# zacharie12/Hypernet-image-captioning

Hardware: AMD Instinct MI355X
Metric: training images/sec at 1/2/4/8 MI355X, Flickr30k GRU+hypernet bs=128 (higher is better)
Workload: dtype f32; 1 GPU; Flickr30k-shaped GRU+additive-attention decoder + hypernet (3 style domains), full training step (fwd, CE, bwd, clip 5.0, Adam); per_gpu_batch=128, global_batch=128, T=20, P=49, D=2048, F=200, E=200, H=200, V=9684, hypernet_params=144906720, parallelism=dp1, launch=eager, next_theta_in_adam_pass=True, next_precompute_beside_adam=True, spinup_steps=0, deterministic_gradients=True

## Files before the change

### hypernet-image-captioning_amd/caphn/_lib.py

```python
import ctypes as C
import os

import torch

_HERE = os.path.dirname(os.path.abspath(__file__))
LIB_PATH = os.environ.get("CAPHN_LIB_PATH") or os.path.join(_HERE, "libcaphn.so")
MAX_HEADS = 8

c_fp = C.c_void_p


class HyperDesc(C.Structure):
    _fields_ = [("he", C.c_int), ("n_heads", C.c_int),
                ("k", C.c_int * MAX_HEADS), ("w", C.c_int * MAX_HEADS),
                ("base_w0", c_fp), ("base_b0", c_fp), ("base_w2", c_fp), ("base_b2", c_fp),
                ("w1", c_fp * MAX_HEADS), ("b1", c_fp * MAX_HEADS),
                ("w2", c_fp * MAX_HEADS), ("b2", c_fp * MAX_HEADS),
                ("d_in", C.c_int), ("d_mid", C.c_int)]


class HyperGrads(C.Structure):
    _fields_ = [("g_base_w0", c_fp), ("g_base_b0", c_fp), ("g_base_w2", c_fp), ("g_base_b2", c_fp),
                ("g_w1", c_fp * MAX_HEADS), ("g_b1", c_fp * MAX_HEADS),
                ("g_w2", c_fp * MAX_HEADS), ("g_b2", c_fp * MAX_HEADS),
# ... 82 lines not shown
    "caphn_colsum_workspace_bytes": (C.c_size_t, [C.c_int, C.c_int]),
    "caphn_linear_wgrad_f32": (C.c_int, [C.c_int, C.c_int, C.c_int, c_fp, C.c_int, c_fp, C.c_int, c_fp, C.c_int, c_fp, c_fp, c_fp]),
    "caphn_colsum_f32": (C.c_int, [C.c_int, C.c_int, c_fp, C.c_int, c_fp, c_fp, c_fp]),
    "caphn_hyper_acts_floats": (C.c_int, [C.POINTER(HyperDesc)]),
    "caphn_hyper_forward": (C.c_int, [C.POINTER(HyperDesc), c_fp, c_fp, c_fp, c_fp]),
    "caphn_hyper_backward_workspace_bytes": (C.c_size_t, [C.POINTER(HyperDesc)]),
    "caphn_hyper_backward": (C.c_int, [C.POINTER(HyperDesc), c_fp, c_fp, C.POINTER(HyperGrads), c_fp, c_fp]),
    "caphn_decoder_workspace_bytes": (C.c_size_t, [C.POINTER(DecoderDims)]),
    "caphn_decoder_forward": (C.c_int, [C.POINTER(DecoderDims), C.POINTER(DecoderParams), c_fp, c_fp,
                                        c_fp, c_fp, c_fp, c_fp]),
    "caphn_decoder_pair_prep": (C.c_int, [C.POINTER(DecoderDims), C.POINTER(DecoderParams), c_fp, c_fp]),
    "caphn_decoder_pair_pack_desc": (C.c_int, [C.POINTER(DecoderDims), c_fp, C.POINTER(PairPack)]),
    "caphn_decoder_precompute": (C.c_int, [C.POINTER(DecoderDims), C.POINTER(DecoderParams), c_fp, c_fp, c_fp, c_fp]),
    "caphn_decoder_inputs": (C.c_int, [C.POINTER(DecoderDims), C.POINTER(DecoderParams), c_fp, c_fp, c_fp]),
    "caphn_decoder_lookup": (C.c_int, [C.POINTER(DecoderDims), C.POINTER(DecoderParams), c_fp, c_fp, c_fp]),
    "caphn_decoder_prepare_rows": (C.c_int, [C.POINTER(DecoderDims), c_fp, C.c_int64, c_fp, c_fp]),
    "caphn_decoder_forward_sampled": (C.c_int, [C.POINTER(DecoderDims), C.POINTER(DecoderParams), c_fp, c_fp,
                                                C.c_char_p, c_fp, c_fp, c_fp, c_fp]),
    "caphn_decoder_forward_sampled_train": (C.c_int, [C.POINTER(DecoderDims), C.POINTER(DecoderParams), c_fp, c_fp,
                                                      C.c_char_p, c_fp, c_fp, c_fp, c_fp]),
    "caphn_decoder_backward": (C.c_int, [C.POINTER(DecoderDims), C.POINTER(DecoderParams), c_fp, c_fp,
                                         c_fp, c_fp, C.POINTER(DecoderGrads), c_fp, c_fp]),
    "caphn_decoder_hyper_backward": (C.c_int, [C.POINTER(DecoderDims), C.POINTER(DecoderParams), c_fp, c_fp,
                                               c_fp, c_fp, C.POINTER(DecoderGrads), c_fp,
                                               C.POINTER(HyperDesc), c_fp, C.POINTER(HyperGrads), c_fp, c_fp]),
    "caphn_decoder_backward_milestone": (C.c_int, [C.c_int, c_fp]),
    "caphn_decoder_search_workspace_bytes": (C.c_size_t, [C.POINTER(DecoderDims), C.POINTER(SearchCfg)]),
    "caphn_decoder_search_begin": (C.c_int, [C.POINTER(DecoderDims), C.POINTER(DecoderParams), C.POINTER(SearchCfg),
                                             c_fp, c_fp, c_fp, c_fp]),
    "caphn_decoder_search_steps": (C.c_int, [C.POINTER(DecoderDims), C.POINTER(DecoderParams), C.POINTER(SearchCfg),
                                             C.c_int, C.c_int, c_fp, c_fp, c_fp, c_fp]),
    "caphn_decoder_search_result": (C.c_int, [C.POINTER(DecoderDims), C.POINTER(SearchCfg), C.c_int, c_fp, c_fp,
                                              c_fp, c_fp, c_fp, c_fp, c_fp, c_fp]),
    "caphn_plain_workspace_bytes": (C.c_size_t, [C.POINTER(PlainDims)]),
    "caphn_plain_forward": (C.c_int, [C.POINTER(PlainDims), C.POINTER(PlainParams), c_fp, c_fp, c_fp, c_fp, c_fp, c_fp, c_fp]),
    "caphn_bahdanau_fwd": (C.c_int, [C.c_int] * 4 + [c_fp] * 8),
    "caphn_bahdanau_bwd": (C.c_int, [C.c_int] * 4 + [c_fp] * 12),
    "caphn_plain_forward_sampled": (C.c_int, [C.POINTER(PlainDims), C.POINTER(PlainParams), c_fp, c_fp, c_fp, C.c_uint64, c_fp, c_fp,
                                               c_fp, c_fp]),
    "caphn_plain_backward": (C.c_int, [C.POINTER(PlainDims), C.POINTER(PlainParams), c_fp, c_fp, c_fp, c_fp, c_fp,
                                       C.POINTER(PlainGrads), c_fp, c_fp]),
    "caphn_layernorm_fwd": (C.c_int, [C.c_int, C.c_int, c_fp, c_fp, c_fp, C.c_float, c_fp, c_fp, c_fp, c_fp]),
    "caphn_layernorm_bwd_workspace_bytes": (C.c_size_t, [C.c_int, C.c_int]),
    "caphn_layernorm_bwd": (C.c_int, [C.c_int, C.c_int, c_fp, c_fp, c_fp, c_fp, c_fp, c_fp, c_fp, c_fp, c_fp, c_fp]),
    "caphn_attention_supported": (C.c_int, [C.POINTER(AttnDims)]),
    "caphn_attention_fwd": (C.c_int, [C.POINTER(AttnDims), c_fp, c_fp, c_fp, c_fp, c_fp, c_fp, c_fp, c_fp]),
    "caphn_attention_bwd": (C.c_int, [C.POINTER(AttnDims), c_fp, c_fp, c_fp, c_fp, c_fp, c_fp, c_fp, c_fp, c_fp, c_fp, c_fp, c_fp]),
    "caphn_ce_workspace_bytes": (C.c_size_t, [C.c_int]),
    "caphn_cross_entropy_rows": (C.c_int, [C.c_int, C.c_int, c_fp, c_fp, C.c_int64, c_fp, C.c_int, c_fp, c_fp, c_fp]),
    "caphn_cross_entropy_rows_ld": (C.c_int, [C.c_int, C.c_int, C.c_int, c_fp, c_fp, C.c_int64, c_fp, C.c_int, c_fp, c_fp, c_fp]),
    "caphn_cross_entropy_finish": (C.c_int, [C.c_int, c_fp, c_fp, c_fp, c_fp]),
    "caphn_decoder_profile_ptr": (C.c_void_p, [C.POINTER(DecoderDims), c_fp]),
    "caphn_decoder_rowcount_ptr": (C.c_void_p, [C.POINTER(DecoderDims), c_fp]),
    "caphn_cross_entropy_fwd_bwd": (C.c_int, [C.c_int, C.c_int, c_fp, c_fp, C.c_int64, c_fp, c_fp, C.c_int, c_fp, c_fp]),
    "caphn_embedding_gather": (C.c_int, [C.c_int, C.c_int, c_fp, c_fp, c_fp, c_fp]),
    "caphn_embedding_scatter_add": (C.c_int, [C.c_int, C.c_int, c_fp, c_fp, c_fp, c_fp]),
    "caphn_embedding_scatter_add_v": (C.c_int, [C.c_int, C.c_int, C.c_int, c_fp, c_fp, c_fp, c_fp]),
    "caphn_sumsq_blocks": (C.c_int, [C.c_size_t]),
    "caphn_sumsq_f32": (C.c_int, [C.c_size_t, c_fp, c_fp, c_fp]),
    "caphn_rank_sumsq_f32": (C.c_int, [C.c_int, C.c_int, C.c_int, c_fp, C.c_size_t, c_fp, C.c_size_t,
                                       c_fp, c_fp, c_fp]),
    "caphn_rank_sumsq_multi_f32": (C.c_int, [C.c_int, C.c_int, C.POINTER(C.c_int), C.POINTER(C.c_int),
                                             C.POINTER(C.c_void_p), C.POINTER(C.c_size_t), C.POINTER(C.c_void_p),
                                             C.POINTER(C.c_size_t), c_fp, c_fp, c_fp]),
    "caphn_grad_norm_workspace_bytes": (C.c_size_t, [C.c_size_t, C.c_int, C.c_int]),
    "caphn_grad_norm_coef": (C.c_int, [C.c_size_t, c_fp, C.c_int, C.c_int, C.POINTER(C.c_int), C.POINTER(C.c_int),
                                       C.POINTER(C.c_void_p), C.POINTER(C.c_size_t), C.POINTER(C.c_void_p),
                                       C.POINTER(C.c_size_t), C.c_double, C.c_double, c_fp, c_fp, c_fp]),
    "caphn_clip_coef": (C.c_int, [C.c_int, c_fp, c_fp, C.c_double, C.c_double, c_fp, c_fp]),
    "caphn_adam_dense_f32": (C.c_int, [C.c_size_t, c_fp, c_fp, c_fp, c_fp, c_fp, C.POINTER(AdamHParams), c_fp]),
    "caphn_grad_norm_adam_dense": (C.c_int, [C.c_size_t, c_fp, c_fp, c_fp, c_fp, C.c_int, C.c_int, C.POINTER(C.c_int), C.POINTER(C.c_int),
                                             C.POINTER(C.c_void_p), C.POINTER(C.c_size_t), C.POINTER(C.c_void_p), C.POINTER(C.c_size_t),
                                             C.c_double, C.c_double, c_fp, c_fp, C.POINTER(AdamHParams), C.c_int, c_fp, c_fp, c_fp, c_fp]),
    "caphn_grad_norm_multi_workspace_bytes": (C.c_size_t, [C.c_int, C.POINTER(C.c_size_t), C.c_int, C.c_int]),
    "caphn_grad_norm_multi": (C.c_int, [C.c_int, C.POINTER(C.c_void_p), C.POINTER(C.c_size_t), C.c_int, C.c_int,
                                        C.POINTER(C.c_int), C.POINTER(C.c_int), C.POINTER(C.c_void_p), C.POINTER(C.c_size_t),
                                        C.POINTER(C.c_void_p), C.POINTER(C.c_size_t), C.c_double, C.c_double, c_fp, c_fp, c_fp]),
    "caphn_adam_multi_f32": (C.c_int, [C.c_int, C.POINTER(C.c_void_p), C.POINTER(C.c_void_p), C.POINTER(C.c_void_p),
                                       C.POINTER(C.c_void_p), C.POINTER(C.c_size_t), c_fp, C.POINTER(AdamHParams), c_fp]),
    "caphn_adam_rank_f32": (C.c_int, [C.c_int, C.c_int, C.c_int, c_fp, c_fp, c_fp, c_fp, C.c_size_t,
                                      c_fp, C.c_size_t, c_fp, C.POINTER(AdamHParams), c_fp]),
    "caphn_adam_rank_gemv_f32": (C.c_int, [C.c_int, C.c_int, C.c_int, c_fp, c_fp, c_fp, c_fp, C.c_size_t,
                                           c_fp, C.c_size_t, c_fp, C.POINTER(AdamHParams), c_fp, c_fp, c_fp, c_fp]),
    "caphn_adam_rank_multi_f32": (C.c_int, [C.c_int, C.c_int, C.POINTER(RankJob), c_fp, C.POINTER(AdamHParams), c_fp]),
    "caphn_hyper_forward_acts": (C.c_int, [C.POINTER(HyperDesc), c_fp, c_fp, c_fp]),
    "caphn_stream_copy_f32": (C.c_int, [C.c_size_t, c_fp, c_fp, c_fp]),
    "caphn_outer_f32": (C.c_int, [C.c_int, C.c_int, c_fp, c_fp, c_fp, c_fp]),
    "caphn_tune": (C.c_int, [C.c_int, C.c_int]),
}

_ERR = {-1: "CAPHN_EINVAL (bad argument)", -2: "CAPHN_ELAUNCH (HIP launch error)",
        -3: "CAPHN_ELIMIT (problem exceeds a hardware limit, e.g. 160 KB LDS)",
        -4: "CAPHN_ETIMEOUT (a recurrent kernel's partner workgroup never answered: that step's results are NaN; "
            "sticky until caphn_device_error(1))"}

_lib = None


class CaphnError(RuntimeError):
    pass


def load():
    global _lib
    if _lib is not None:
        return _lib
# ... 34 lines not shown
```

### hypernet-image-captioning_amd/caphn/ops.py

```python
import ctypes as C
from dataclasses import dataclass
from typing import Dict, List, Optional, Sequence, Tuple

import torch

from . import _lib as L

GEMM_BIAS, GEMM_RELU, GEMM_ACCUM, GEMM_MASK, GEMM_LRELU = 1, 2, 4, 8, 16


def _f32(*shape, device):
    return torch.empty(*shape, dtype=torch.float32, device=device)


def gemm(a: torch.Tensor, b: torch.Tensor, ta: bool = False, tb: bool = False,
         bias: Optional[torch.Tensor] = None, relu: bool = False, out: Optional[torch.Tensor] = None,
         accumulate: bool = False, mask: Optional[torch.Tensor] = None, splitk: int = 1, lrelu: bool = False) -> torch.Tensor:
    lib = L.load()
    assert a.dim() == 2 and b.dim() == 2 and a.stride(1) == 1 and b.stride(1) == 1
    M, K = (a.shape[1], a.shape[0]) if ta else (a.shape[0], a.shape[1])
    N, Kb = (b.shape[0], b.shape[1]) if tb else (b.shape[1], b.shape[0])
    if K != Kb:
        raise L.CaphnError(f"gemm inner dims differ: {K} vs {Kb}")
    if out is None:
# ... 522 lines not shown
    lib = L.load()
    cd = dims.c()
    ps = _dec_struct(L.DecoderParams, dims, params)
    gs = _dec_struct(L.DecoderGrads, dims, grads)
    L.check(lib.caphn_decoder_backward(C.byref(cd), C.byref(ps), L.ptr(features), L.ptr(captions, torch.int64),
                                       L.ptr(dlogits), L.ptr(dalphas, allow_none=True), C.byref(gs),
                                       C.c_void_p(ws.data_ptr()), L.stream_ptr()), "caphn_decoder_backward")


def cross_entropy_fwd_bwd(logits: torch.Tensor, targets: torch.Tensor, ignore_index: int = 0,
                          dlogits: Optional[torch.Tensor] = None, leave_ignored_rows: bool = False):
    lib = L.load()
    V = logits.shape[-1]
    rows = logits.numel() // V
    if dlogits is None:
        dlogits = torch.empty_like(logits)
    ws = torch.empty(lib.caphn_ce_workspace_bytes(rows), dtype=torch.uint8, device=logits.device)
    out = _f32(2, device=logits.device)
    L.check(lib.caphn_cross_entropy_fwd_bwd(rows, V, L.ptr(logits), L.ptr(targets.reshape(-1), torch.int64),
                                            ignore_index, L.ptr(dlogits), L.ptr(out), int(leave_ignored_rows),
                                            C.c_void_p(ws.data_ptr()),
                                            L.stream_ptr()), "caphn_cross_entropy_fwd_bwd")
    return out, dlogits


def cross_entropy_rows(logits: torch.Tensor, targets: torch.Tensor, ignore_index: int, dlogits: torch.Tensor,
                       ws: torch.Tensor, leave_ignored_rows: bool = False, n_valid_ptr: Optional[int] = None, V: Optional[int] = None) -> None:
    lib = L.load()
    ld = logits.shape[-1]
    rows = logits.numel() // ld
    V = ld if V is None else int(V)
    assert dlogits.shape[-1] == ld and V <= ld
    L.check(lib.caphn_cross_entropy_rows_ld(rows, V, ld, L.ptr(logits), L.ptr(targets.reshape(-1), torch.int64), ignore_index,
                                            L.ptr(dlogits), int(leave_ignored_rows),
                                            C.c_void_p(n_valid_ptr) if n_valid_ptr else None, C.c_void_p(ws.data_ptr()),
                                            L.stream_ptr()), "caphn_cross_entropy_rows_ld")


def cross_entropy_finish(rows: int, ws: torch.Tensor, out: torch.Tensor, n_valid_ptr: Optional[int] = None) -> None:
    lib = L.load()
    L.check(lib.caphn_cross_entropy_finish(rows, C.c_void_p(n_valid_ptr) if n_valid_ptr else None, L.ptr(out),
                                           C.c_void_p(ws.data_ptr()), L.stream_ptr()), "caphn_cross_entropy_finish")


def ce_workspace(rows: int, device) -> torch.Tensor:
    return torch.empty(L.load().caphn_ce_workspace_bytes(rows), dtype=torch.uint8, device=device)


def decoder_rowcount_ptr(dims: DecDims, ws: torch.Tensor) -> int:
    cd = dims.c()
    return int(L.load().caphn_decoder_rowcount_ptr(C.byref(cd), C.c_void_p(ws.data_ptr())) or 0)


def embedding_gather(table: torch.Tensor, idx: torch.Tensor) -> torch.Tensor:
    lib = L.load()
    rows, E = idx.numel(), table.shape[1]
    out = _f32(rows, E, device=table.device)
    L.check(lib.caphn_embedding_gather(rows, E, L.ptr(table), L.ptr(idx.reshape(-1), torch.int64), L.ptr(out),
                                       L.stream_ptr()), "caphn_embedding_gather")
    return out


def embedding_scatter_add(g: torch.Tensor, idx: torch.Tensor, table_grad: torch.Tensor) -> None:
    lib = L.load()
    rows, E = g.shape
    L.check(lib.caphn_embedding_scatter_add_v(rows, E, int(table_grad.shape[0]), L.ptr(g), L.ptr(idx.reshape(-1), torch.int64),
                                              L.ptr(table_grad), L.stream_ptr()), "caphn_embedding_scatter_add_v")


def sumsq_partials(x: torch.Tensor, partial: Optional[torch.Tensor] = None) -> torch.Tensor:
    lib = L.load()
    nb = lib.caphn_sumsq_blocks(x.numel())
    if partial is None:
        partial = torch.empty(nb, dtype=torch.float64, device=x.device)
    L.check(lib.caphn_sumsq_f32(x.numel(), L.ptr(x), L.ptr(partial, torch.float64), L.stream_ptr()), "caphn_sumsq_f32")
    return partial[:nb]


def rank_sumsq(gfac: torch.Tensor, afac: torch.Tensor, acc: torch.Tensor) -> None:
    lib = L.load()
    R, rows = gfac.shape
    k = afac.shape[1]
    ws = torch.empty(2 * R * R, dtype=torch.float64, device=gfac.device)
    L.check(lib.caphn_rank_sumsq_f32(R, rows, k, gfac.data_ptr(), gfac.stride(0), afac.data_ptr(), afac.stride(0),
                                     L.ptr(acc, torch.float64), L.ptr(ws, torch.float64), L.stream_ptr()),
            "caphn_rank_sumsq_f32")


def rank_sumsq_multi(pairs, acc: torch.Tensor, ws: Optional[torch.Tensor] = None) -> None:
    lib = L.load()
    n = len(pairs)
    R = pairs[0][0].shape[0]
    if ws is None:
        ws = torch.empty(2 * R * R * n, dtype=torch.float64, device=acc.device)
    rows = (C.c_int * n)(*[g.shape[1] for g, _ in pairs])
    ks = (C.c_int * n)(*[a.shape[1] for _, a in pairs])
    gp = (C.c_void_p * n)(*[g.data_ptr() for g, _ in pairs])
    ap = (C.c_void_p * n)(*[a.data_ptr() for _, a in pairs])
    ldg = (C.c_size_t * n)(*[g.stride(0) for g, _ in pairs])
    lda = (C.c_size_t * n)(*[a.stride(0) for _, a in pairs])
    L.check(lib.caphn_rank_sumsq_multi_f32(R, n, rows, ks, gp, ldg, ap, lda, L.ptr(acc, torch.float64),
                                           L.ptr(ws, torch.float64), L.stream_ptr()), "caphn_rank_sumsq_multi_f32")


class GradNorm:

# ... 409 lines not shown
```

### hypernet-image-captioning_amd/csrc/decoder.hip

```cpp
#include "common.h"
#include "decoder_internal.h"
#include "gemm_internal.h"
#include <algorithm>
#include <initializer_list>
#include <mutex>

int g_tune_deterministic = 0;
int g_tune_rec_pair = 1;
int g_tune_rec_rotate = 1;
int g_tune_vocab_order = 1;
int g_tune_branch_mask = 7;
int g_tune_splitk_target = 1280;
int g_tune_chain_main = 0;
int g_tune_hops = 0;
int g_tune_fork = 4;
int g_tune_join_chain = 0;
int g_tune_sk_dhs = 0, g_tune_sk_vocab_w = 0;
#define RUN(x) do { int _rc = (x); if (_rc != CAPHN_OK) return _rc; } while (0)

namespace {

struct Side {
    hipStream_t st[3];
    enum { D_FORK = 0, D_JOIN = 1, D_X = 4, D_MS = 10, D_PRE_F = 14, D_PRE_ALL = 15, D_COUNT = 16 };
    struct Dep { hipEvent_t ev; unsigned seq = 0; bool by_value = false; };
    Dep deps[D_COUNT];
    unsigned* vals = nullptr;
    unsigned counter = 0;
    bool values = false;
    bool pre_valid = false;
    const void* pre_ws = nullptr;
    bool ready = false, on = false;
    bool forked[3] = {false, false, false};
    hipStream_t main = nullptr;
    int init() {
        if (ready) return CAPHN_OK;
        static std::mutex mu;
        std::lock_guard<std::mutex> lock(mu);
        if (ready) return CAPHN_OK;
        for (auto& s : st) if (hipStreamCreateWithFlags(&s, hipStreamNonBlocking) != hipSuccess) return CAPHN_ELAUNCH;
        for (auto& d : deps) if (hipEventCreateWithFlags(&d.ev, hipEventDisableTiming) != hipSuccess) return CAPHN_ELAUNCH;
        void* p = nullptr;
        if (hipMalloc(&p, sizeof(unsigned) * D_COUNT) == hipSuccess && hipMemset(p, 0, sizeof(unsigned) * D_COUNT) == hipSuccess)
            vals = static_cast<unsigned*>(p);
        else (void)hipGetLastError();
        ready = true;
        return CAPHN_OK;
    }
    int post(int slot, hipStream_t from) {
        Dep& d = deps[slot];
        if (values) {
            d.seq = ++counter; d.by_value = true;
            return hipStreamWriteValue32(from, vals + slot, d.seq, 0) == hipSuccess ? CAPHN_OK : CAPHN_ELAUNCH;
        }
        d.by_value = false;
        return hipEventRecord(d.ev, from) == hipSuccess ? CAPHN_OK : CAPHN_ELAUNCH;
    }
    int await(int slot, hipStream_t to) {
        Dep& d = deps[slot];
        if (d.by_value)
            return hipStreamWaitValue32(to, vals + slot, d.seq, hipStreamWaitValueGte, 0xffffffffu) == hipSuccess ? CAPHN_OK : CAPHN_ELAUNCH;
        return hipStreamWaitEvent(to, d.ev, 0) == hipSuccess ? CAPHN_OK : CAPHN_ELAUNCH;
    }
    int milestone(int k, hipStream_t from) {
        if (init() != CAPHN_OK) return CAPHN_ELAUNCH;
        return post(D_MS + k, from);
    }
    int begin(hipStream_t m, bool enable) {
// ... 16 lines not shown
        if (post(D_FORK, main) != CAPHN_OK) return CAPHN_ELAUNCH;
        for (int i : ids) {
            if (!((g_tune_branch_mask >> i) & 1)) continue;
            if (await(D_FORK, st[i]) != CAPHN_OK) return CAPHN_ELAUNCH;
            forked[i] = true;
        }
        return CAPHN_OK;
    }
    int jointo(int i) {
        if (!on || !((g_tune_branch_mask >> i) & 1)) return CAPHN_OK;
        forked[i] = false;
        if (post(D_JOIN + i, st[i]) != CAPHN_OK) return CAPHN_ELAUNCH;
        return await(D_JOIN + i, main);
    }
    int join_into(int i, int j) {
        if (!on || !((g_tune_branch_mask >> i) & 1)) return CAPHN_OK;
        if (!((g_tune_branch_mask >> j) & 1)) return jointo(i);
        forked[i] = false;
        if (post(D_JOIN + i, st[i]) != CAPHN_OK) return CAPHN_ELAUNCH;
        return await(D_JOIN + i, st[j]);
    }
    struct Scope {
        Side& s;
        explicit Scope(Side& side) : s(side) {}
        ~Scope() { for (int i = 0; i < 3; ++i) if (s.on && s.forked[i]) (void)s.jointo(i); }
    };
    hipStream_t xfrom[6] = {nullptr, nullptr, nullptr, nullptr, nullptr, nullptr};
    int record(int k, hipStream_t from) {
        if (!on) return CAPHN_OK;
        xfrom[k] = from;
        return post(D_X + k, from);
    }
    int wait(int k, hipStream_t to) {
        if (!on || xfrom[k] == to) return CAPHN_OK;
        return await(D_X + k, to);
    }
    int dep(hipStream_t from, hipStream_t to, int k) {
        if (!on || from == to) return CAPHN_OK;
        if (post(D_X + k, from) != CAPHN_OK) return CAPHN_ELAUNCH;
        return await(D_X + k, to);
    }
};
constexpr int MAX_DEVICES = 64;
Side g_sides[MAX_DEVICES];
inline Side* side_here() {
    int dev = 0;
    if (hipGetDevice(&dev) != hipSuccess || dev < 0 || dev >= MAX_DEVICES) return nullptr;
    return &g_sides[dev];
}

struct Ws {
    size_t Y1, f, meanf, h0, c0, Waf, G, Xe, Xg, Hs, Hprev, gates, hn, Cs, Cprev, uah, alphas, idx;
    size_t dHs, dgi, dgh, duah, de, dh0, dc0, ctx, dctx, dXe, dWaf, dmeanf, df, dY1, apart, vtmp, colws, colws_s[3], prof, rowmap;
    size_t xch, xch_floats;
    size_t wp;
    size_t H0s, dH0, h0L, dcarry, tgi, tgh, tmpA, tmpB;
    size_t Lin[CAPHN_MAX_DEC_LAYERS - 1], Lgates[CAPHN_MAX_DEC_LAYERS - 1], Lhn[CAPHN_MAX_DEC_LAYERS - 1],
           Ldgi[CAPHN_MAX_DEC_LAYERS - 1], Ldgh[CAPHN_MAX_DEC_LAYERS - 1];
    int L1;
    size_t total;
    int npc, pchunk, NG, arows;
};
inline bool use_pair(const caphn_decoder_dims* d) {
    const int NG = d->cell == CAPHN_CELL_LSTM ? 4 : 3;
    return g_tune_rec_pair && d->T > 1 && d->layers <= 1 && caphn_rec_pair_resident_gates(d->P, d->H, NG) >= 0;
}

inline size_t up4(size_t v) { return (v + 3) & ~(size_t)3; }

inline Ws layout(const caphn_decoder_dims* d) {
    Ws w;
    const size_t B = d->B, T = d->T, P = d->P, F = d->F, E = d->E, H = d->H, V = d->V, D = d->D;
    const bool lstm = d->cell == CAPHN_CELL_LSTM, raw = d->raw_features != 0;
    const size_t NG = lstm ? 4 : 3;
    w.NG = (int)NG;
    size_t o = 0;
    auto take = [&](size_t n) { size_t r = o; o += up4(n); return r; };
    w.Y1 = take(raw ? 0 : B * P * F); w.f = take(raw ? 0 : B * P * F); w.meanf = take(B * F); w.h0 = take(B * H);
    w.c0 = take(lstm ? B * H : 0);
    w.Waf = take(B * P * H); w.G = take(B * P * NG * H); w.Xe = take(B * T * (E + F)); w.Xg = take(B * T * NG * H);
    w.Hs = take(B * T * H); w.Hprev = take(B * T * H); w.gates = take(B * T * NG * H); w.hn = take(lstm ? 0 : B * T * H);
    w.Cs = take(lstm ? B * T * H : 0); w.Cprev = take(lstm ? B * T * H : 0);
    w.uah = take(B * T * H); w.alphas = take(B * T * P); w.idx = take(2 * B * T);
    w.dHs = take(B * T * H); w.dgi = take(B * T * NG * H); w.dgh = take(lstm ? 0 : B * T * NG * H); w.duah = take(B * T * H);
    w.de = take(B * T * P); w.dh0 = take(B * H); w.dc0 = take(lstm ? B * H : 0);
    w.ctx = w.Xe + E; w.dctx = take(raw ? 0 : B * T * F);
    w.dXe = take(B * T * E); w.dWaf = take(B * P * H); w.dmeanf = take(raw ? 0 : 2 * B * F); w.df = take(raw ? 0 : B * P * F);
    w.dY1 = take(raw ? 0 : B * P * F);
    w.pchunk = 1; w.npc = (int)((P + w.pchunk - 1) / w.pchunk);
    const size_t arows = std::max<size_t>(std::max<size_t>(w.npc, (size_t)caphn_rec_bwd_groups((int)P, (int)H)),
                                          (size_t)caphn_rec_pair_bwd_groups((int)P, (int)H));
    w.arows = (int)arows;
    w.apart = take(B * arows * (H + 1)); w.vtmp = take(H + 1);
    size_t cs = 0;
    auto need = [&](size_t M, size_t N) { cs = std::max(cs, caphn_colsum_workspace_bytes((int)M, (int)N) / sizeof(float)); };
    need(B * T, V); need(B * T, NG * H); need(B * T, H); need(B * P, H); need(B * P, F); need(B, H);
    need(B * arows, H + 1);
    if (d->layers > 1) need(B * (T + 1), 3 * H);
    w.colws = take(cs);
    {
        size_t c2 = 0;
        auto need2 = [&](size_t M, size_t N) { c2 = std::max(c2, caphn_colsum_workspace_bytes((int)M, (int)N) / sizeof(float)); };
        need2(B * T, NG * H); need2(B * T, H); need2(B * P, H); need2(B * P, F); need2(B, H); need2(B * arows, H + 1);
        if (d->layers > 1) need2(B * (T + 1), 3 * H);
        for (int i = 0; i < 3; ++i) w.colws_s[i] = take(c2);
    }
    w.prof = take(64);
    w.rowmap = take(B * T + 4);
    w.xch_floats = caphn_rec_pair_xch_bytes((int)B, (int)P, (int)H) / sizeof(float);
    w.xch = take(2 * w.xch_floats);
    o = (o + 31) & ~(size_t)31;
    w.wp = take(caphn_rec_pair_wp_floats((int)H, (int)NG));
    w.L1 = d->layers > 1 ? d->layers - 1 : 0;
    {
        const size_t on = w.L1 > 0 ? 1 : 0, S = T + 1;
        w.H0s = take(on * B * T * H); w.dH0 = take(on * B * T * H); w.h0L = take(on * B * H); w.dcarry = take(on * B * H);
        w.tgi = take(on * B * 3 * H); w.tgh = take(on * B * 3 * H); w.tmpA = take(on * B * H); w.tmpB = take(on * B * H);
        for (int l = 0; l < CAPHN_MAX_DEC_LAYERS - 1; ++l) {
            const size_t u = l < w.L1 ? 1 : 0;
            w.Lin[l] = take(u * B * S * H); w.Lgates[l] = take(u * B * S * 3 * H); w.Lhn[l] = take(u * B * S * H);
            w.Ldgi[l] = take(u * B * S * 3 * H); w.Ldgh[l] = take(u * B * S * 3 * H);
        }
    }
    w.total = o;
    (void)D;
    return w;
}

__global__ __launch_bounds__(1024) void valid_rows_kernel(int n, const int64_t* __restrict__ tgt, int64_t ignore, int* __restrict__ map) {
    __shared__ int wsum[16];
    __shared__ int base_s;
    const int tid = threadIdx.x, lane = tid & 63, wave = tid >> 6;
    if (tid == 0) base_s = 0;
    __syncthreads();
    for (int c0 = 0; c0 < n; c0 += 1024) {
        const int i = c0 + tid;
        const int v = (i < n && tgt[i] != ignore) ? 1 : 0;
        const unsigned long long ball = __ballot(v);
        const int before = __popcll(ball & ((1ull << lane) - 1ull));
        if (lane == 0) wsum[wave] = __popcll(ball);
        __syncthreads();
        int woff = 0, tot = 0;
        for (int q = 0; q < 16; ++q) { if (q < wave) woff += wsum[q]; tot += wsum[q]; }
        const int base = base_s;
        if (v) map[4 + base + woff + before] = i;
        __syncthreads();
        if (tid == 0) base_s = base + tot;
        __syncthreads();
    }
    if (tid == 0) map[0] = base_s;
}

__global__ void copy2_kernel(const float* __restrict__ src, int n, float* __restrict__ a, float* __restrict__ b) {
    const int i = blockIdx.x * blockDim.x + threadIdx.x;
    if (i < n) a[i] = src[i];
    else if (i == n) b[0] = src[n];
}

__global__ __launch_bounds__(256) void teacher_inputs_kernel(int T, int E, const int64_t* __restrict__ caps, const float* __restrict__ table,
                                                            int64_t* __restrict__ idx, float* __restrict__ out, int ostride) {
    const int i = blockIdx.x, t = i % T;
    const int64_t id = t < 2 ? (int64_t)-1 : caps[i - 1];
    if (threadIdx.x == 0) idx[i] = id;
    for (int e = threadIdx.x; e < E; e += 256) out[(size_t)i * ostride + e] = id < 0 ? 0.f : table[(size_t)id * E + e];
}

inline bool dims_ok(const caphn_decoder_dims* d) {
    if (d && !(d->dropout_p >= 0.f && d->dropout_p < 1.f)) return false;
    if (!(d && d->B > 0 && d->T > 0 && d->P > 0 && d->D > 0 && d->F > 0 && d->E > 0 && d->H > 0 && d->V > 0)) return false;
    if (d->cell != CAPHN_CELL_GRU && d->cell != CAPHN_CELL_LSTM) return false;
    if (d->raw_features && d->F != d->D) return false;
    if (d->layers < 0 || d->layers > CAPHN_MAX_DEC_LAYERS) return false;
    if (d->layers > 1 && d->cell != CAPHN_CELL_GRU) return false;
    if (d->logits_ld != 0 && d->logits_ld < d->V) return false;
    return true;
}
inline bool layer_params_ok(const caphn_decoder_dims* d, const caphn_decoder_params* p) {
    for (int l = 0; l + 1 < d->layers; ++l)
        if (!p->lw_ih[l] || !p->lw_hh[l] || !p->lb_ih[l] || !p->lb_hh[l]) return false;
    return true;
}

inline int pick_splitk(int M, int N, int K) {
    if (g_tune_deterministic) return 1;
    const long t128 = (long)((M + 127) / 128) * ((N + 127) / 128);
    if (t128 >= 1024) return 1;
    const long t64 = (long)((M + 63) / 64) * ((N + 63) / 64);
    const int nslab = (K + 31) / 32;
    long s = (g_tune_splitk_target + t64 - 1) / t64;
    if (s > nslab / 8) s = nslab / 8;
    if (s < 1) s = 1;
    if (s > 64) s = 64;
    return (int)s;
}


inline int gemm_auto(int ta, int tb, int M, int N, int K, const float* A, int lda, const float* B, int ldb,
                     float* C, int ldc, const float* bias, int flags, hipStream_t s,
                     const int* rowmap = nullptr, int map_mode = 0, bool prezeroed = false) {
    int sk = pick_splitk(M, N, K);
    if (rowmap) {
        if (sk > 1 && !prezeroed) {
            if (ldc == N) { RUN(caphn_zero_f32(C, (size_t)M * N, s)); }
// ... 80 lines not shown
    const int B = d->B, H = d->H, G3 = 3 * d->H;
    const float* in = hin; int in_ld = hin_ld;
    for (int l = 0; l < w.L1; ++l) {
        const bool last = l == w.L1 - 1;
        float* out = last ? hout : ws + ((l & 1) ? w.tmpB : w.tmpA);
        const int out_ld = last ? hout_ld : H;
        RUN(caphn_gemm_f32(0, 1, B, G3, H, in, in_ld, p->lw_ih[l], H, ws + w.tgi, G3, p->lb_ih[l], nullptr, 0, CAPHN_GEMM_BIAS, 1, s));
        RUN(caphn_gemm_f32(0, 1, B, G3, H, in, in_ld, p->lw_hh[l], H, ws + w.tgh, G3, p->lb_hh[l], nullptr, 0, CAPHN_GEMM_BIAS, 1, s));
        LayerFwdArgs a;
        a.B = B; a.H = H; a.S = d->T + 1; a.slot = slot;
        a.gi = ws + w.tgi; a.gh = ws + w.tgh; a.hin = in; a.hin_ld = in_ld; a.hout = out; a.hout_ld = out_ld;
        a.sin = ws + w.Lin[l]; a.sgates = ws + w.Lgates[l]; a.shn = ws + w.Lhn[l];
        if (last && slot > 0) { a.drop_p = d->dropout_p; a.drop_seed = d->dropout_seed; a.T = d->T; a.t = slot - 1; }
        RUN(caphn_launch_layer_gru_fwd(a, s));
        in = out; in_ld = out_ld;
    }
    return CAPHN_OK;
}

static int layers_backward(const caphn_decoder_dims* d, const caphn_decoder_params* p, const Ws& w, float* ws, int slot,
                           const float* d1, int d1_ld, const float* d2, float* dout, int dout_ld, hipStream_t s) {
    const int B = d->B, H = d->H, G3 = 3 * d->H, S = d->T + 1;
    for (int l = w.L1 - 1; l >= 0; --l) {
        float* o = l == 0 ? dout : ws + ((l & 1) ? w.tmpB : w.tmpA);
        const int o_ld = l == 0 ? dout_ld : H;
        LayerBwdArgs a;
        a.B = B; a.H = H; a.S = S; a.slot = slot;
        a.d1 = d1; a.d1_ld = d1_ld; a.d2 = d2;
        a.sin = ws + w.Lin[l]; a.sgates = ws + w.Lgates[l]; a.shn = ws + w.Lhn[l];
        a.dgi = ws + w.Ldgi[l]; a.dgh = ws + w.Ldgh[l]; a.dout = o; a.dout_ld = o_ld;
        if (l == w.L1 - 1 && slot > 0) { a.drop_p = d->dropout_p; a.drop_seed = d->dropout_seed; a.T = d->T; a.t = slot - 1; }
        RUN(caphn_launch_layer_gru_bwd(a, s));
        RUN(caphn_gemm_f32(0, 0, B, H, G3, ws + w.Ldgi[l] + (size_t)slot * G3, S * G3, p->lw_ih[l], H, o, o_ld, nullptr, nullptr, 0,
                           CAPHN_GEMM_ACCUM, 1, s));
        RUN(caphn_gemm_f32(0, 0, B, H, G3, ws + w.Ldgh[l] + (size_t)slot * G3, S * G3, p->lw_hh[l], H, o, o_ld, nullptr, nullptr, 0,
                           CAPHN_GEMM_ACCUM, 1, s));
        d1 = o; d1_ld = o_ld; d2 = nullptr;
    }
    return CAPHN_OK;
}

}

extern "C" size_t caphn_decoder_workspace_bytes(const caphn_decoder_dims* d) {
    if (!dims_ok(d)) return 0;
    return layout(d).total * sizeof(float);
}

extern "C" const int* caphn_decoder_rowcount_ptr(const caphn_decoder_dims* d, void* ws_) {
    if (!dims_ok(d) || !ws_) return nullptr;
    return reinterpret_cast<const int*>(static_cast<float*>(ws_) + layout(d).rowmap);
}

extern "C" unsigned long long* caphn_decoder_profile_ptr(const caphn_decoder_dims* d, void* ws_) {
    if (!dims_ok(d) || !ws_) return nullptr;
    return reinterpret_cast<unsigned long long*>(static_cast<float*>(ws_) + layout(d).prof);
}

extern "C" int caphn_decoder_prepare_rows(const caphn_decoder_dims* d, const int64_t* targets, int64_t ignore_index,
                                          void* ws_, caphn_stream_t stream) {
    if (!dims_ok(d) || !targets || !ws_) return CAPHN_EINVAL;
    const Ws w = layout(d);
    hipLaunchKernelGGL(valid_rows_kernel, dim3(1), dim3(1024), 0, static_cast<hipStream_t>(stream), d->B * d->T, targets,
                       ignore_index, reinterpret_cast<int*>(static_cast<float*>(ws_) + w.rowmap));
    return caphn_launch_status();
}

static int decoder_inputs(const caphn_decoder_dims* d, const caphn_decoder_params* p, const Ws& w, float* ws,
                          const int64_t* captions, hipStream_t s, int parts = 3) {
    const int BT = d->B * d->T, E = d->E, GH = w.NG * d->H, EF = d->E + d->F;
    int64_t* idx = reinterpret_cast<int64_t*>(ws + w.idx);
    if ((parts & 1) && !(d->precomputed & 64))
        hipLaunchKernelGGL(teacher_inputs_kernel, dim3(BT), dim3(256), 0, s, d->T, E, captions, p->embed_w, idx, ws + w.Xe, EF);
    if (parts & 2)
    RUN(caphn_gemm_f32(0, 1, BT, GH, E, ws + w.Xe, EF, p->w_ih, EF, ws + w.Xg, GH, p->b_ih, nullptr, 0, CAPHN_GEMM_BIAS, 1, s));
    return CAPHN_OK;
}

extern "C" int caphn_decoder_precompute(const caphn_decoder_dims* d, const caphn_decoder_params* p, const float* features,
                                        const int64_t* captions, void* ws_, caphn_stream_t stream) {
    if (!dims_ok(d) || !p || !features || !ws_) return CAPHN_EINVAL;
    const bool raw = d->raw_features != 0;
    if (!raw && (!p->fc0_w || !p->fc0_b || !p->fc2_w || !p->fc2_b)) return CAPHN_EINVAL;
    if (d->cell == CAPHN_CELL_LSTM && (!p->initc_w || !p->initc_b)) return CAPHN_EINVAL;
    const Ws w = layout(d);
    hipStream_t s = static_cast<hipStream_t>(stream);
    const float* f = nullptr;
    RUN(decoder_precompute(d, p, w, static_cast<float*>(ws_), features, &f, s, (captions ? 3 : 1) & ~(d->precomputed & 1), true));
    if (captions && !(d->precomputed & 4)) RUN(decoder_inputs(d, p, w, static_cast<float*>(ws_), captions, s));
    Side* sd = side_here();
    if (!sd || sd->post(Side::D_PRE_ALL, s) != CAPHN_OK) return CAPHN_ELAUNCH;
    sd->pre_valid = true;
    sd->pre_ws = ws_;
    return caphn_launch_status();
}

extern "C" int caphn_decoder_pair_prep(const caphn_decoder_dims* d, const caphn_decoder_params* p, void* ws_, caphn_stream_t stream) {
    if (!dims_ok(d) || !p || !ws_ || !p->Ua_w || !use_pair(d)) return CAPHN_EINVAL;
    const Ws w = layout(d);
    float* ws = static_cast<float*>(ws_);
    RUN(caphn_launch_rec_pair_prep(reinterpret_cast<unsigned long long*>(ws + w.xch), 2 * w.xch_floats * sizeof(float) / sizeof(unsigned long long),
                                   p->Ua_w, nullptr, d->H, w.NG, ws + w.wp, ws + w.dHs, (size_t)d->B * d->T * d->H,
                                   static_cast<hipStream_t>(stream)));
    return caphn_launch_status();
}
extern "C" int caphn_decoder_pair_pack_desc(const caphn_decoder_dims* d, void* ws_, caphn_pair_pack* out) {
    if (!dims_ok(d) || !ws_ || !out || !use_pair(d)) return CAPHN_EINVAL;
    const Ws w = layout(d);
    out->wp = static_cast<float*>(ws_) + w.wp;
    out->H = d->H; out->HA = caphn_rec_pair_half_a(d->H); out->pitch = caphn_rec_pair_pitch(d->H);
    out->hrows = (w.NG + 1) * out->HA;
    return CAPHN_OK;
}

extern "C" int caphn_decoder_inputs(const caphn_decoder_dims* d, const caphn_decoder_params* p, const int64_t* captions,
                                    void* ws_, caphn_stream_t stream) {
    if (!dims_ok(d) || !p || !captions || !ws_ || !p->embed_w || !p->w_ih || !p->b_ih) return CAPHN_EINVAL;
    const Ws w = layout(d);
    RUN(decoder_inputs(d, p, w, static_cast<float*>(ws_), captions, static_cast<hipStream_t>(stream)));
    return caphn_launch_status();
}
extern "C" int caphn_decoder_lookup(const caphn_decoder_dims* d, const caphn_decoder_params* p, const int64_t* captions,
                                    void* ws_, caphn_stream_t stream) {
    if (!dims_ok(d) || !p || !captions || !ws_ || !p->embed_w) return CAPHN_EINVAL;
    const Ws w = layout(d);
    RUN(decoder_inputs(d, p, w, static_cast<float*>(ws_), captions, static_cast<hipStream_t>(stream), 1));
    return caphn_launch_status();
}

extern "C" int caphn_decoder_forward(const caphn_decoder_dims* d, const caphn_decoder_params* p,
                                     const float* features, const int64_t* captions,
                                     float* logits, float* alphas, void* ws_, caphn_stream_t stream) {
    if (!dims_ok(d) || !p || !features || !captions || !logits || !ws_) return CAPHN_EINVAL;
    hipStream_t s = static_cast<hipStream_t>(stream);
    const Ws w = layout(d);
    float* ws = static_cast<float*>(ws_);
    const int B = d->B, T = d->T, P = d->P, D = d->D, F = d->F, E = d->E, H = d->H, V = d->V;
    const bool lstm = d->cell == CAPHN_CELL_LSTM, raw = d->raw_features != 0;
    const int BP = B * P, BT = B * T, GH = w.NG * H, EF = E + F;
    const bool pair = use_pair(d);
    const int RG = pair ? caphn_rec_pair_resident_gates(P, H, w.NG) : caphn_rec_resident_gates(P, H, w.NG);
    if (RG < 0) return CAPHN_ELIMIT;
    if (lstm && (!p->initc_w || !p->initc_b)) return CAPHN_EINVAL;
    if (!raw && (!p->fc0_w || !p->fc0_b || !p->fc2_w || !p->fc2_b)) return CAPHN_EINVAL;
    if (!layer_params_ok(d, p)) return CAPHN_EINVAL;

    const float* f = nullptr;
    const int pc = d->precomputed;
    if (!(pc & 4)) RUN(decoder_inputs(d, p, w, ws, captions, s));
    Side* sdw = (pc & 16) ? side_here() : nullptr;
    if (pc & 16) {
        if (!sdw || !sdw->pre_valid || sdw->pre_ws != ws_) return CAPHN_EINVAL;
        RUN(sdw->await(Side::D_PRE_F, s));
    }
    RUN(decoder_precompute(d, p, w, ws, features, &f, s, ((pc & 1) ? 0 : 1) | ((pc & 2) ? 0 : 2)));
    if (pc & 16)
        RUN(sdw->await(Side::D_PRE_ALL, s));

    RecFwdArgs a;
    a.B = B; a.T = T; a.P = P; a.H = H; a.RG = RG;
    a.Waf = ws + w.Waf; a.G = ws + w.G; a.Xg = ws + w.Xg; a.h0 = ws + w.h0; a.c0 = ws + w.c0;
    a.W_hh = p->w_hh; a.b_hh = p->b_hh; a.U_a = p->Ua_w; a.b_Ua = p->Ua_b; a.v_a = p->va_w; a.b_va = p->va_b;
    a.Hs = ws + w.Hs; a.Hprev = ws + w.Hprev; a.alphas = ws + w.alphas; a.gates = ws + w.gates; a.hn = ws + w.hn;
    a.Cs = ws + w.Cs; a.Cprev = ws + w.Cprev; a.uah = ws + w.uah;
    a.vecW = (H % 4 == 0) && caphn_aligned16(p->w_hh) && caphn_aligned16(p->Ua_w);
    a.vecS = (H % 4 == 0) && caphn_aligned16(ws);
    a.prof = reinterpret_cast<unsigned long long*>(ws + w.prof);
    a.rotate = g_tune_rec_rotate;
    a.drop_p = d->dropout_p; a.drop_seed = d->dropout_seed;
    if (pair) {
        a.xch = reinterpret_cast<unsigned long long*>(ws + w.xch);
        a.WP = ws + w.wp; a.wp_pitch = caphn_rec_pair_pitch(H);
        if (!(pc & 128))
        RUN(caphn_launch_rec_pair_prep(a.xch, 2 * w.xch_floats * sizeof(float) / sizeof(unsigned long long), p->Ua_w, p->w_hh, H, w.NG,
                                       ws + w.wp, (pc & 8) ? ws + w.dHs : nullptr, (size_t)BT * H, s));
        RUN(caphn_launch_rec_pair_fwd(a, lstm, s));
    } else if (w.L1 > 0) {
        RUN(layers_forward(d, p, w, ws, 0, ws + w.h0, H, ws + w.h0L, H, s));
        a.h0 = ws + w.h0L; a.Hs = ws + w.H0s; a.Hsrc = ws + w.Hs; a.drop_p = 0.f;
        for (int t = 0; t < T; ++t) {
            a.t0 = t; a.t1 = t + 1;
            RUN(caphn_launch_rec_fwd(a, lstm, s));
            RUN(layers_forward(d, p, w, ws, t + 1, ws + w.H0s + (size_t)t * H, T * H, ws + w.Hs + (size_t)t * H, T * H, s));
        }
    } else
    RUN(caphn_launch_rec_fwd(a, lstm, s));
    if ((pc & 8) && !pair) RUN(caphn_zero_f32(ws + w.dHs, (size_t)BT * H, s));

    const int LV = d->logits_ld > 0 ? d->logits_ld : V;
    if (d->row_subset)
        RUN(caphn_gemm_mapped(0, 1, BT, V, H, ws + w.Hs, H, p->out_w, H, logits, LV, p->out_b, CAPHN_GEMM_BIAS, 1,
                              reinterpret_cast<const int*>(ws + w.rowmap) + 4, reinterpret_cast<const int*>(ws + w.rowmap), 1, s));
    else
        RUN(caphn_gemm_f32(0, 1, BT, V, H, ws + w.Hs, H, p->out_w, H, logits, LV, p->out_b, nullptr, 0, CAPHN_GEMM_BIAS, 1, s));
    if (pc & 32) RUN(caphn_launch_ctx(B, T, P, F, ws + w.alphas, f, ws + w.ctx, EF, s));
    if (alphas)
        if (hipMemcpyAsync(alphas, ws + w.alphas, sizeof(float) * (size_t)BT * P, hipMemcpyDeviceToDevice, s) != hipSuccess)
            return CAPHN_ELAUNCH;
    return caphn_launch_status();
}

struct HyperHook { const caphn_hyper_desc* hd; const float* acts; const caphn_hyper_grads* hg; void* ws; };
static int decoder_backward_impl(const caphn_decoder_dims* d, const caphn_decoder_params* p,
                                 const float* features, const int64_t* captions, float* dlogits, const float* dalphas,
                                 const caphn_decoder_grads* g, void* ws_, const HyperHook* hook, caphn_stream_t stream);
extern "C" int caphn_decoder_backward(const caphn_decoder_dims* d, const caphn_decoder_params* p,
                                      const float* features, const int64_t* captions,
                                      float* dlogits, const float* dalphas,
                                      const caphn_decoder_grads* g, void* ws_, caphn_stream_t stream) {
    return decoder_backward_impl(d, p, features, captions, dlogits, dalphas, g, ws_, nullptr, stream);
}
extern "C" int caphn_decoder_hyper_backward(const caphn_decoder_dims* d, const caphn_decoder_params* p,
                                            const float* features, const int64_t* captions,
                                            float* dlogits, const float* dalphas,
                                            const caphn_decoder_grads* g, void* ws_,
                                            const caphn_hyper_desc* hd, const float* acts, const caphn_hyper_grads* hg, void* hyper_ws,
                                            caphn_stream_t stream) {
    if (!hd || !acts || !hg || !hyper_ws || !g) return CAPHN_EINVAL;
    const size_t NG = d && d->cell == CAPHN_CELL_LSTM ? 4 : 3;
    if (d) {
        const size_t GH = NG * d->H, EF = (size_t)d->E + d->F;
        if (g->w_hh != g->w_ih + GH * EF || g->b_ih != g->w_hh + GH * d->H || g->b_hh != g->b_ih + GH) return CAPHN_EINVAL;
    }
    HyperHook hook{hd, acts, hg, hyper_ws};
    return decoder_backward_impl(d, p, features, captions, dlogits, dalphas, g, ws_, &hook, stream);
}
static int decoder_backward_impl(const caphn_decoder_dims* d, const caphn_decoder_params* p,
                                 const float* features, const int64_t* captions, float* dlogits, const float* dalphas,
                                 const caphn_decoder_grads* g, void* ws_, const HyperHook* hook, caphn_stream_t stream) {
    if (!dims_ok(d) || !p || !features || !captions || !dlogits || !g || !ws_) return CAPHN_EINVAL;
    hipStream_t s = static_cast<hipStream_t>(stream);
    const Ws w = layout(d);
    float* ws = static_cast<float*>(ws_);
    const int B = d->B, T = d->T, P = d->P, D = d->D, F = d->F, E = d->E, H = d->H, V = d->V;
    const bool lstm = d->cell == CAPHN_CELL_LSTM, raw = d->raw_features != 0;
    const int BP = B * P, BT = B * T, GH = w.NG * H, EF = E + F;
    const bool pair = use_pair(d);
    const int RG = pair ? caphn_rec_pair_resident_gates(P, H, w.NG) : caphn_rec_resident_gates(P, H, w.NG);
    if (RG < 0) return CAPHN_ELIMIT;
    if (lstm && (!g->initc_w || !g->initc_b)) return CAPHN_EINVAL;
    if (!raw && (!g->fc0_w || !g->fc0_b || !g->fc2_w || !g->fc2_b)) return CAPHN_EINVAL;
    if (!layer_params_ok(d, p)) return CAPHN_EINVAL;
    for (int l = 0; l < w.L1; ++l) if (!g->lw_ih[l] || !g->lw_hh[l] || !g->lb_ih[l] || !g->lb_hh[l]) return CAPHN_EINVAL;
    void* cws = ws + w.colws;
    const int64_t* idx = reinterpret_cast<const int64_t*>(ws + w.idx);
    const float* f = raw ? features : ws + w.f;
    float* dgi = ws + w.dgi;
    float* dgh = lstm ? dgi : ws + w.dgh;

    Side* sdp = side_here();
    if (!sdp) return CAPHN_ELAUNCH;
    Side& sd = *sdp;
    RUN(sd.begin(s, g_tune_fork != 0));
    Side::Scope scope(sd);
    void* cw0 = ws + w.colws_s[0]; void* cw1 = ws + w.colws_s[1]; void* cw2 = ws + w.colws_s[2];

    const int* rmap = d->row_subset ? reinterpret_cast<const int*>(ws + w.rowmap) : nullptr;
    const int LV = d->logits_ld > 0 ? d->logits_ld : V;
    const int fork_mode = g_tune_fork == 4 ? (pair ? 2 : 1) : g_tune_fork;
    const bool late = fork_mode != 2;
    const bool gz = d->grads_zeroed != 0;
    const bool wg_first = !late && g_tune_vocab_order == 0;
    if (wg_first) {
        RUN(sd.forkto(0));
        RUN(wgrad_bias(V, H, BT, dlogits, LV, ws + w.Hs, H, g->out_w, H, g->out_b, rmap, cws, sd.s(0), gz));
        RUN(sd.milestone(CAPHN_MS_VOCAB, sd.s(0)));
    }
    const bool dhs_zero = (d->precomputed & 8) != 0;
    bool ctx_side = false;
    if (rmap) {
        if (!dhs_zero) RUN(caphn_zero_f32(ws + w.dHs, (size_t)BT * H, s));
        RUN(caphn_gemm_mapped(0, 0, BT, H, V, dlogits, LV, p->out_w, H, ws + w.dHs, H, nullptr, 0,
                              (g_tune_sk_dhs > 0 && !g_tune_deterministic) ? g_tune_sk_dhs : pick_splitk(BT, H, V),
                              rmap + 4, rmap, 1, s));
    } else
    RUN(gemm_auto(0, 0, BT, H, V, dlogits, LV, p->out_w, H, ws + w.dHs, H, nullptr, 0, s, nullptr, 0, dhs_zero));
    if (!late && !wg_first) {
        if (!(d->precomputed & 32) && sd.s(0) != s && sd.s(2) != s) {
            RUN(sd.fork_many({0, 2}));
            RUN(caphn_launch_ctx(B, T, P, F, ws + w.alphas, f, ws + w.ctx, EF, sd.s(2)));
            RUN(sd.record(5, sd.s(2)));
            ctx_side = true;
        } else
        RUN(sd.forkto(0));
        RUN(wgrad_bias(V, H, BT, dlogits, LV, ws + w.Hs, H, g->out_w, H, g->out_b, rmap, cws, sd.s(0), gz));
        RUN(sd.milestone(CAPHN_MS_VOCAB, sd.s(0)));
    }

    RecBwdArgs a;
    a.B = B; a.T = T; a.P = P; a.H = H; a.RG = RG;
    a.Waf = ws + w.Waf; a.G = ws + w.G; a.W_hh = p->w_hh; a.U_a = p->Ua_w; a.v_a = p->va_w;
    a.Hprev = ws + w.Hprev; a.alphas = ws + w.alphas; a.gates = ws + w.gates; a.hn = ws + w.hn; a.uah = ws + w.uah;
    a.Cs = ws + w.Cs; a.Cprev = ws + w.Cprev;
    a.dHs = ws + w.dHs; a.dalphas = dalphas;
    a.dgi = dgi; a.dgh = dgh; a.duah = ws + w.duah; a.de = ws + w.de; a.dh0 = ws + w.dh0; a.dc0 = ws + w.dc0;
    a.vecW = (H % 4 == 0) && caphn_aligned16(p->w_hh) && caphn_aligned16(p->Ua_w);
    a.vecS = (H % 4 == 0) && caphn_aligned16(ws);
    a.prof = reinterpret_cast<unsigned long long*>(ws + w.prof) + 8;
    a.rotate = g_tune_rec_rotate;
    a.drop_p = d->dropout_p; a.drop_seed = d->dropout_seed;
    const int ang = w.L1 > 0 ? 0 : pair ? caphn_rec_pair_bwd_groups(P, H) : caphn_rec_bwd_groups(P, H);
    if (ang > 0) { a.dWaf = ws + w.dWaf; a.apart = ws + w.apart; }
    if (w.L1 > 0) {
        RUN(caphn_zero_f32(ws + w.dcarry, (size_t)B * H, s));
        a.dHs = ws + w.dH0; a.dh0 = ws + w.dcarry; a.drop_p = 0.f;
        for (int t = T - 1; t >= 0; --t) {
            RUN(layers_backward(d, p, w, ws, t + 1, ws + w.dHs + (size_t)t * H, T * H, ws + w.dcarry, ws + w.dH0 + (size_t)t * H, T * H, s));
            a.t0 = t; a.t1 = t + 1;
            RUN(caphn_launch_rec_bwd(a, lstm, s));
        }
        RUN(layers_backward(d, p, w, ws, 0, ws + w.dcarry, H, nullptr, ws + w.dh0, H, s));
    } else if (pair) {
        a.xch = reinterpret_cast<unsigned long long*>(ws + w.xch) + w.xch_floats * sizeof(float) / sizeof(unsigned long long);
        a.apart_rows = ang;
        a.WP = ws + w.wp; a.wp_pitch = caphn_rec_pair_pitch(H);
        if (!raw) { a.inith_w = p->inith_w; a.initc_w = lstm ? p->initc_w : nullptr; a.dmean_part = ws + w.dmeanf; a.F = F; }
        RUN(caphn_launch_rec_pair_bwd(a, lstm, s));
    } else
    RUN(caphn_launch_rec_bwd(a, lstm, s));

    hipStream_t b0 = sd.s(0), b1 = sd.s(1), b2 = sd.s(2);
    const bool t_main = hook != nullptr && g_tune_chain_main != 0;
    hipStream_t sT = t_main ? s : b1, sF = t_main ? b1 : s;
    const bool hold_big = late && !raw && fork_mode == 3;
    RUN(sd.fork_many({0, 1, 2}));
    if (late && !hold_big) {
        RUN(wgrad_bias(V, H, BT, dlogits, LV, ws + w.Hs, H, g->out_w, H, g->out_b, rmap, cws, b0, gz));
        RUN(sd.milestone(CAPHN_MS_VOCAB, b0));
    }
    if (ctx_side) RUN(sd.wait(5, sT));
    else if (!(d->precomputed & 32)) RUN(caphn_launch_ctx(B, T, P, F, ws + w.alphas, f, ws + w.ctx, EF, sT));
    if (lstm) RUN(gemm_auto(1, 0, GH, EF, BT, dgi, GH, ws + w.Xe, EF, g->w_ih, EF, nullptr, 0, sT, nullptr, 0, gz));
    else RUN(wgrad_bias(GH, EF, BT, dgi, GH, ws + w.Xe, EF, g->w_ih, EF, g->b_ih, nullptr, cw1, sT, gz));
    RUN(wgrad_bias(GH, H, BT, dgh, GH, ws + w.Hprev, H, g->w_hh, H, g->b_hh, nullptr, cw2, b2, gz));
    if (lstm) RUN(caphn_colsum_f32(BT, GH, dgi, GH, g->b_ih, cw2, b2));
    RUN(sd.record(3, b2));
    hipStream_t se = late ? b2 : b0;
    RUN(caphn_gemm_f32(0, 0, BT, E, GH, dgi, GH, p->w_ih, EF, ws + w.dXe, E, nullptr, nullptr, 0, 0, 1, se));
    if (!gz) RUN(caphn_zero_f32(g->embed_w, (size_t)V * E, se));
    RUN(caphn_embedding_scatter_add_v(BT, E, V, ws + w.dXe, idx, g->embed_w, se));
    RUN(sd.milestone(CAPHN_MS_EMBED, se));
    RUN(sd.wait(3, sT));
    RUN(sd.milestone(CAPHN_MS_DTHETA, sT));
    if (hook && !hold_big) {
        RUN(caphn_hyper_backward(hook->hd, g->w_ih, hook->acts, hook->hg, hook->ws, sT));
    }
    if (!hold_big) RUN(sd.milestone(CAPHN_MS_HYPER, sT));
    if (!raw) {
        RUN(caphn_gemm_f32(0, 0, BT, F, GH, dgi, GH, p->w_ih + E, EF, ws + w.dctx, F, nullptr, nullptr, 0, 0, 1, sF));
        if (!pair)
            RUN(caphn_launch_dmean(B, H, F, ws + w.dh0, p->inith_w, lstm ? ws + w.dc0 : nullptr, lstm ? p->initc_w : nullptr,
                                   ws + w.dmeanf, sF));
    }
    AttnGradArgs ag;
    ag.T = T; ag.P = P; ag.H = H; ag.pchunk = w.pchunk;
    ag.Waf = ws + w.Waf; ag.uah = ws + w.uah; ag.de = ws + w.de; ag.v_a = p->va_w;
    ag.dWaf = ws + w.dWaf; ag.part = ws + w.apart;
    if (ang == 0) RUN(caphn_launch_attn_param_grads(ag, B, w.npc, sF));
    RUN(sd.record(2, sF));
    RUN(wgrad_bias(H, H, BT, ws + w.duah, H, ws + w.Hprev, H, g->Ua_w, H, g->Ua_b, nullptr, cws, b0, gz));
    for (int l = 0; l < w.L1; ++l) {
        const int BS = B * (T + 1), G3 = 3 * H;
        RUN(wgrad_bias(G3, H, BS, ws + w.Ldgi[l], G3, ws + w.Lin[l], H, g->lw_ih[l], H, g->lb_ih[l], nullptr, cws, b0, gz));
        RUN(wgrad_bias(G3, H, BS, ws + w.Ldgh[l], G3, ws + w.Lin[l], H, g->lw_hh[l], H, g->lb_hh[l], nullptr, cws, b0, gz));
    }
    RUN(wgrad_bias(H, F, B, ws + w.dh0, H, ws + w.meanf, F, g->inith_w, F, g->inith_b, nullptr, cws, b0, gz));
    if (lstm) RUN(wgrad_bias(H, F, B, ws + w.dc0, H, ws + w.meanf, F, g->initc_w, F, g->initc_b, nullptr, cws, b0, gz));
    if (!raw) {
        RUN(caphn_launch_df(B, T, P, F, ws + w.alphas, ws + w.dctx, ws + w.dmeanf, ws + w.df, sF, pair ? ws + w.dmeanf + (size_t)B * F : nullptr));
        RUN(caphn_gemm_f32(0, 0, BP, F, H, ws + w.dWaf, H, p->Wa_w, F, ws + w.df, F, nullptr, nullptr, 0, CAPHN_GEMM_ACCUM, 1, sF));
        RUN(sd.record(4, sF));
        if (hold_big) {
            RUN(sd.wait(4, b0));
            RUN(wgrad_bias(V, H, BT, dlogits, LV, ws + w.Hs, H, g->out_w, H, g->out_b, rmap, cws, b0, gz));
            RUN(sd.milestone(CAPHN_MS_VOCAB, b0));
            if (hook) {
                RUN(sd.wait(4, sT));
                RUN(caphn_hyper_backward(hook->hd, g->w_ih, hook->acts, hook->hg, hook->ws, sT));
            }
            RUN(sd.milestone(CAPHN_MS_HYPER, sT));
        }
        RUN(caphn_gemm_f32(0, 0, BP, F, F, ws + w.df, F, p->fc2_w, F, ws + w.dY1, F, nullptr, ws + w.Y1, F, CAPHN_GEMM_MASK, 1, sF));
        RUN(wgrad_bias(F, D, BP, ws + w.dY1, F, features, D, g->fc0_w, D, g->fc0_b, nullptr, cw0, sF, gz));
    }
    RUN(sd.wait(2, b2));
    RUN(caphn_colsum_f32(B * (ang > 0 ? ang : w.npc), H + 1, ws + w.apart, H + 1, ws + w.vtmp, cw2, b2));
    hipLaunchKernelGGL(copy2_kernel, dim3((H + 256) / 256), dim3(256), 0, b2, ws + w.vtmp, H, g->va_w, g->va_b);
    RUN(wgrad_bias(H, F, BP, ws + w.dWaf, H, f, F, g->Wa_w, F, g->Wa_b, nullptr, cw2, b2, gz));
    if (!raw) {
        RUN(sd.wait(4, b2));
        RUN(wgrad_bias(F, F, BP, ws + w.df, F, ws + w.Y1, F, g->fc2_w, F, g->fc2_b, nullptr, cw2, b2, gz));
    }
    if (g_tune_join_chain) { RUN(sd.join_into(0, 1)); RUN(sd.join_into(2, 1)); RUN(sd.jointo(1)); }
    else { RUN(sd.jointo(0)); RUN(sd.jointo(1)); RUN(sd.jointo(2)); }
    (void)captions;
    return caphn_launch_status();
}

extern "C" int caphn_decoder_backward_milestone(int which, caphn_stream_t waiter) {
    if (which < 0 || which >= CAPHN_MS_COUNT) return CAPHN_EINVAL;
    Side* sd = side_here();
    if (!sd) return CAPHN_ELAUNCH;
    if (!sd->ready) return CAPHN_OK;
    return sd->await(Side::D_MS + which, static_cast<hipStream_t>(waiter));
}

extern "C" int caphn_decoder_forward_sampled(const caphn_decoder_dims* d, const caphn_decoder_params* p,
                                             const float* features, const int64_t* captions,
                                             const unsigned char* use_sampling,
                                             float* logits, float* alphas, void* ws_, caphn_stream_t stream) {
    if (!dims_ok(d) || !p || !features || !captions || !use_sampling || !logits || !ws_ || d->logits_ld != 0) return CAPHN_EINVAL;
    if (d->dropout_p > 0.f) return CAPHN_EINVAL;
    hipStream_t s = static_cast<hipStream_t>(stream);
    const Ws w = layout(d);
    float* ws = static_cast<float*>(ws_);
    const int B = d->B, T = d->T, P = d->P, E = d->E, F = d->F, H = d->H, V = d->V;
    const bool lstm = d->cell == CAPHN_CELL_LSTM;
    const int GH = w.NG * H, EF = E + F;
    const int RG = caphn_rec_resident_gates(P, H, w.NG);
    if (RG < 0) return CAPHN_ELIMIT;
    if (lstm && (!p->initc_w || !p->initc_b)) return CAPHN_EINVAL;
    const float* f = nullptr;
// ... 215 lines not shown
```

### hypernet-image-captioning_amd/csrc/decoder_internal.h

```cpp
#pragma once
#include "common.h"

struct RecFwdArgs {
    int B, T, P, H;
    int RG;
    const float* Waf;
    const float* G;
    const float* Xg;
    const float* h0;
    const float* c0;
    const float* W_hh; const float* b_hh;
    const float* U_a; const float* b_Ua;
    const float* v_a; const float* b_va;
    float* Hs; float* Hprev;
    float* alphas;
    float* gates;
    float* hn;
    float* Cs; float* Cprev;
    float* uah;
    unsigned long long* prof;
    int vecW, vecS, rotate;
    int slab_div = 1;
    unsigned long long* xch = nullptr;
    const float* WP = nullptr; int wp_pitch = 0;
    int t0 = 0, t1 = 0;
    float drop_p = 0.f; unsigned long long drop_seed = 0;
    int waf_lds = 0;
    int wc_rows = 0;
    unsigned epoch = 0; int* err = nullptr; long long xlimit = 0;
    const float* Hsrc = nullptr;
};
struct RecBwdArgs {
    int B, T, P, H;
    int RG;
    const float* Waf; const float* G;
    const float* W_hh; const float* U_a; const float* v_a;
    const float* Hprev; const float* alphas; const float* gates; const float* hn; const float* uah;
    const float* Cs; const float* Cprev;
    const float* dHs;
    const float* dalphas;
    float* dgi; float* dgh;
    float* duah;
    float* de;
    float* dh0;
    float* dc0;
    unsigned long long* prof;
    int vecW, vecS, rotate;
    float* dWaf = nullptr; float* apart = nullptr;
    unsigned long long* xch = nullptr;
    const float* WP = nullptr; int wp_pitch = 0;
    int apart_rows = 0;
    float drop_p = 0.f; unsigned long long drop_seed = 0;
    unsigned epoch = 0; int* err = nullptr; long long xlimit = 0;
    const float* inith_w = nullptr; const float* initc_w = nullptr; float* dmean_part = nullptr; int F = 0;
    int part_rows = 0, wc_rows = 0;
    int t0 = 0, t1 = 0;
};
struct AttnGradArgs {
    int T, P, H, pchunk;
    const float* Waf; const float* uah; const float* de; const float* v_a;
    float* dWaf;
    float* part;
};

struct LayerFwdArgs {
    int B, H, S, slot;
    const float* gi; const float* gh;
    const float* hin; int hin_ld;
    float* hout; int hout_ld;
    float* sin; float* sgates; float* shn;
    float drop_p = 0.f; unsigned long long drop_seed = 0; int T = 1, t = 0;
};
struct LayerBwdArgs {
    int B, H, S, slot;
    const float* d1; int d1_ld; const float* d2;
    const float* sin; const float* sgates; const float* shn;
    float* dgi; float* dgh;
    float* dout; int dout_ld;
    float drop_p = 0.f; unsigned long long drop_seed = 0; int T = 1, t = 0;
};
int caphn_launch_layer_gru_fwd(const LayerFwdArgs& a, hipStream_t s);
int caphn_launch_layer_gru_bwd(const LayerBwdArgs& a, hipStream_t s);

size_t caphn_rec_fwd_lds_bytes(int P, int H, int NG, int RG);
size_t caphn_rec_bwd_lds_bytes(int P, int H, int NG, int RG);
int caphn_rec_resident_gates(int P, int H, int NG);
int caphn_launch_rec_fwd(const RecFwdArgs& a, bool lstm, hipStream_t s);
int caphn_launch_rec_bwd(const RecBwdArgs& a, bool lstm, hipStream_t s);
bool caphn_rec_pair_ok(int P, int H, int NG, int RG);
int caphn_rec_pair_resident_gates(int P, int H, int NG);
size_t caphn_rec_pair_xch_bytes(int B, int P, int H);
int caphn_rec_pair_bwd_groups(int P, int H);
int caphn_rec_pair_pitch(int H);
int caphn_rec_pair_half_a(int H);
size_t caphn_rec_pair_wp_floats(int H, int NG);
int caphn_launch_rec_pair_prep(unsigned long long* xch, size_t nxch, const float* U_a, const float* W_hh, int H, int NG, float* WP,
                               float* zbuf, size_t nz, hipStream_t s);
int caphn_launch_rec_pair_fwd(const RecFwdArgs& a, bool lstm, hipStream_t s);
int caphn_launch_rec_pair_bwd(const RecBwdArgs& a, bool lstm, hipStream_t s);
int caphn_rec_bwd_groups(int P, int H);
int caphn_launch_attn_param_grads(const AttnGradArgs& a, int B, int npc, hipStream_t s);
int caphn_launch_ctx(int B, int T, int P, int F, const float* alphas, const float* f, float* ctx, int ldc, hipStream_t s);
int caphn_launch_df(int B, int T, int P, int F, const float* alphas, const float* dctx, const float* dmean, float* df, hipStream_t s,
                    const float* dmean2 = nullptr);
int caphn_launch_dmean(int B, int H, int F, const float* dh0, const float* Wh, const float* dc0, const float* Wc, float* out, hipStream_t s);
int caphn_launch_init_state(int B, int P, int F, int H, const float* f, const float* Wh, const float* bh, const float* Wc,
                            const float* bc, float* meanf, float* h0, float* c0, hipStream_t s);
int caphn_embedding_gather_strided(int rows, int E, const float* table, const int64_t* idx, int istride, float* out, int ostride, hipStream_t s);
int caphn_launch_mean_p(int B, int P, int F, const float* f, float* out, hipStream_t s);

constexpr int SEARCH_MAX_BEAM = 8;
struct SearchArgs {
    int n_images, beam, max_steps, H;
    int zero_pad_rule;
    int64_t end_token;
    float* h_cur; const float* h_new;
    float* score;
    int64_t* idx;
    const float* cand_val; const int* cand_idx;
    int* k_alive; int* n_comp;
    int64_t* seqs[2];
    int64_t* comp_seqs; int* comp_len; float* comp_score;
};
int caphn_launch_row_topk(int R, int V, int k, const float* logits, const float* score, float* cand_val, int* cand_idx, hipStream_t s);
int caphn_launch_beam_merge(const SearchArgs& a, int step, hipStream_t s);
int caphn_launch_search_init(const SearchArgs& a, const float* h0, int64_t first_token, int lookup_first, hipStream_t s);
int caphn_launch_search_result(const SearchArgs& a, int steps_done, int64_t* out_seq, int* out_len, float* out_score, int* finished,
                               int* n_active, hipStream_t s);
```

### hypernet-image-captioning_amd/csrc/hyper.hip

```cpp
#include "common.h"
#include <algorithm>

namespace {

constexpr float LRELU = 0.01f;
__device__ __forceinline__ float lrelu(float v) { return v > 0.f ? v : LRELU * v; }
__device__ __forceinline__ float lrelu_grad(float post) { return post > 0.f ? 1.f : LRELU; }

struct GemvJob {
    const float* W; const float* b; const float* x; float* y;
    int rows, k, act, vec;
    int block0, nblocks;
    float* xcopy;
};
struct GemvJobs { GemvJob j[CAPHN_MAX_HEADS]; int n; };

template <int QMAX, int RB, bool NTL>
__device__ __forceinline__ void gemv_rows_wave(const GemvJob& J, int wave_g, int nwaves, int lane) {
    const int k4 = J.k >> 2;
    const f32x4* x4 = reinterpret_cast<const f32x4*>(J.x);
    f32x4 xr[QMAX];
#pragma unroll
    for (int q = 0; q < QMAX; ++q) {
        int c = lane + 64 * q;
// ... 775 lines not shown
            if (!out) return;
            OuterJob& J = oj.j[oj.n++];
            J.g = gv; J.a = av; J.out = out; J.rows = rows; J.k = k; J.block0 = b0;
            b0 += ((long)rows * k + 1023) / 1024;
        };
        add(ws + W.dzb0, acts + L.x, g->g_base_w0, d_mid(d), d_in(d));
        add(ws + W.dzb2, acts + L.a0, g->g_base_w2, d->he, d_mid(d));
        for (int i = 0; i < nh; ++i) add(ws + W.dz[i], acts + L.base, g->g_w1[i], d->k[i], d->he);
        if (oj.n) hipLaunchKernelGGL(outer_kernel, dim3((unsigned)b0), dim3(256), 0, s, oj);
        for (int i = 0; i < nh; ++i)
            if (g->g_w2[i]) {
                OuterJobs o2; o2.n = 1;
                OuterJob& J = o2.j[0];
                J.g = dtheta + toff[i]; J.a = acts + L.a[i]; J.out = g->g_w2[i]; J.rows = d->w[i]; J.k = d->k[i]; J.block0 = 0;
                long nb = ((long)J.rows * J.k + 1023) / 1024;
                hipLaunchKernelGGL(outer_kernel, dim3((unsigned)nb), dim3(256), 0, s, o2);
            }
    }
    return caphn_launch_status();
}

extern "C" int caphn_outer_f32(int rows, int k, const float* gv, const float* av, float* out, caphn_stream_t stream) {
    if (rows <= 0 || k <= 0 || !gv || !av || !out) return CAPHN_EINVAL;
    OuterJobs o2; o2.n = 1;
    OuterJob& J = o2.j[0];
    J.g = gv; J.a = av; J.out = out; J.rows = rows; J.k = k; J.block0 = 0;
    long nb = ((long)rows * k + 1023) / 1024;
    hipLaunchKernelGGL(outer_kernel, dim3((unsigned)nb), dim3(256), 0, static_cast<hipStream_t>(stream), o2);
    return caphn_launch_status();
}

extern int g_tune_adam;
extern int g_tune_gemm;
extern int g_tune_rec_rotate;
extern int g_tune_fork;
extern int g_tune_gemm_xcd;
extern int g_tune_gemm_fast;
extern int g_tune_gemm_planes;
extern int g_tune_rec_pair;
extern int g_tune_gemm_single;
extern int g_tune_gemm_tile;
extern int g_tune_deterministic;
extern int g_tune_adam_cap;
extern int g_tune_chain_main;
extern int g_tune_rec_cache;
extern int g_tune_splitk_target;
extern int g_tune_gemm_order;
extern int g_tune_branch_mask;
extern int g_tune_gemm_db;
extern int g_tune_gemm_ws;
extern int g_tune_adam_dense_cap;
extern int g_tune_sk_dhs, g_tune_sk_vocab_w;
extern int g_tune_join_chain;
extern int g_tune_gemm_kres;
extern int g_tune_gemm_waves;
extern int g_tune_hops;
extern int g_tune_vocab_order;
extern int g_det_vocab;
int caphn_rec_pair_debug_skip(int v);
int caphn_rec_pair_debug_opts(int v);
extern "C" int caphn_tune(int key, int value) {
    if (key == 0) { g_tune_gemv = value; return CAPHN_OK; }
    if (key == 1) { g_tune_adam = value; return CAPHN_OK; }
    if (key == 2) { g_tune_gemm = value; return CAPHN_OK; }
    if (key == 3) { g_tune_rec_rotate = value; return CAPHN_OK; }
    if (key == 4) { g_tune_fork = value; return CAPHN_OK; }
    if (key == 6) { g_tune_gemm_xcd = value; return CAPHN_OK; }
    if (key == 7) { g_tune_gemm_fast = value; return CAPHN_OK; }
    if (key == 8) { g_tune_gemm_planes = value; return CAPHN_OK; }
    if (key == 9) { g_tune_rec_pair = value; return CAPHN_OK; }
    if (key == 10) return caphn_rec_pair_debug_skip(value);
    if (key == 11) { g_tune_gemm_single = value; return CAPHN_OK; }
    if (key == 12) { g_tune_gemm_tile = value; return CAPHN_OK; }
    if (key == 13) { g_tune_deterministic = value > 0; g_det_vocab = value; return CAPHN_OK; }
    if (key == 21) { g_tune_vocab_order = value != 0; return CAPHN_OK; }
    if (key == 20) { if (value < 0 || value > 7) return CAPHN_EINVAL; g_tune_branch_mask = value; return CAPHN_OK; }
    if (key == 18) { if (value < 0 || value > 2) return CAPHN_EINVAL; g_tune_gemm_order = value; return CAPHN_OK; }
    if (key == 17) { if (value < 1 || value > 65536) return CAPHN_EINVAL; g_tune_splitk_target = value; return CAPHN_OK; }
    if (key == 16) { if (value < 0 || value > 2) return CAPHN_EINVAL; g_tune_rec_cache = value; return CAPHN_OK; }
    if (key == 15) { g_tune_chain_main = value != 0; return CAPHN_OK; }
    if (key == 26) { g_tune_hops = value != 0; return CAPHN_OK; }
    if (key == 27) { g_tune_hyper_tail = value != 0; return CAPHN_OK; }
    if (key == 28) { g_tune_acts_fused = value != 0; return CAPHN_OK; }
    if (key == 36) { g_tune_gemm_kres = value != 0; return CAPHN_OK; }
    if (key == 35) { g_tune_join_chain = value != 0; return CAPHN_OK; }
    if (key == 33) { if (value < 0 || value > 64) return CAPHN_EINVAL; g_tune_sk_dhs = value; return CAPHN_OK; }
    if (key == 34) { if (value < 0 || value > 64) return CAPHN_EINVAL; g_tune_sk_vocab_w = value; return CAPHN_OK; }
    if (key == 30) { if (value < 64 || value > 4096) return CAPHN_EINVAL; g_tune_vjp_blocks = value; return CAPHN_OK; }
    if (key == 31) { if (value < 64 || value > 65535) return CAPHN_EINVAL; g_tune_adam_dense_cap = value; return CAPHN_OK; }
    if (key == 29) { if (value != 0 && value != 64 && value != 128) return CAPHN_EINVAL; g_tune_gemm_ws = value; return CAPHN_OK; }
    if (key == 25) { if (value != 0 && value != 5 && value != 6) return CAPHN_EINVAL; g_tune_gemm_waves = value; return CAPHN_OK; }
    if (key == 24) return caphn_rec_pair_debug_opts(value);
    if (key == 23) { if (value < 0 || value > 7) return CAPHN_EINVAL; g_tune_gemm_db = value; return CAPHN_OK; }
    if (key == 22) { if (value < 1) return CAPHN_EINVAL; g_tune_xch_timeout = 100ll * value; return CAPHN_OK; }
    if (key == 14) { if (value < 64 || value > 65535) return CAPHN_EINVAL; g_tune_adam_cap = value; return CAPHN_OK; }
    return CAPHN_EINVAL;
}
```

### hypernet-image-captioning_amd/csrc/misc.hip

```cpp
#include "common.h"
#include "gemm_internal.h"
#include <math.h>

namespace {
constexpr int RMAX = 8;


__global__ __launch_bounds__(256) void ce_count_kernel(int rows, const int64_t* __restrict__ tgt, int64_t ignore, float* nvalid) {
    __shared__ int cnt[4];
    int c = 0;
    for (int i = threadIdx.x; i < rows; i += 256) c += (tgt[i] != ignore);
    float cf = wave_sum((float)c);
    if ((threadIdx.x & 63) == 0) cnt[threadIdx.x >> 6] = (int)cf;
    __syncthreads();
    if (threadIdx.x == 0) nvalid[0] = (float)(cnt[0] + cnt[1] + cnt[2] + cnt[3]);
}

__global__ __launch_bounds__(256) void ce_row_kernel(int V, int ld, const float* logits, const int64_t* __restrict__ tgt,
                                                     int64_t ignore, const float* __restrict__ nvalid, const int* __restrict__ nvi,
                                                     float* dlogits, float* __restrict__ row_loss, int vec) {
    __shared__ float red[4];
    __shared__ float bc[2];
    const int row = blockIdx.x, tid = threadIdx.x;
    const float* x = logits + (size_t)row * ld;
// ... 143 lines not shown
}

__global__ __launch_bounds__(256) void scale_kernel(size_t n, const float* __restrict__ x, const float* __restrict__ scale, float* __restrict__ out) {
    const float c = scale[0];
    const size_t stride = (size_t)gridDim.x * 256;
    for (size_t i = (size_t)blockIdx.x * 256 + threadIdx.x; i < n; i += stride) out[i] = x[i] * c;
}

__global__ __launch_bounds__(256) void lrelu_bwd_kernel(size_t n, const float* __restrict__ dy, const float* __restrict__ post, float* __restrict__ dx) {
    for (size_t i = (size_t)blockIdx.x * 256 + threadIdx.x; i < n; i += (size_t)gridDim.x * 256) dx[i] = dy[i] * (post[i] > 0.f ? 1.f : 0.01f);
}
__global__ __launch_bounds__(256) void axpy_kernel(size_t n, float alpha, const float* __restrict__ x, float* __restrict__ y) {
    const size_t stride = (size_t)gridDim.x * 256;
    for (size_t i = (size_t)blockIdx.x * 256 + threadIdx.x; i < n; i += stride) y[i] = fmaf(alpha, x[i], y[i]);
}

__global__ __launch_bounds__(256) void colsum_kernel(int M, int N, const float* __restrict__ A, int lda,
                                                     float* __restrict__ out, int rows_per) {
    __shared__ float red[4][65];
    const int c = threadIdx.x & 63, rl = threadIdx.x >> 6;
    const int n = blockIdx.x * 64 + c;
    const int m0 = blockIdx.y * rows_per, m1 = min(M, m0 + rows_per);
    float s0 = 0.f, s1 = 0.f;
    if (n < N) {
        int m = m0 + rl;
        for (; m + 4 < m1; m += 8) { s0 += A[(size_t)m * lda + n]; s1 += A[(size_t)(m + 4) * lda + n]; }
        if (m < m1) s0 += A[(size_t)m * lda + n];
    }
    red[rl][c] = s0 + s1;
    __syncthreads();
    if (rl == 0 && n < N) out[(size_t)blockIdx.y * N + n] = (red[0][c] + red[1][c]) + (red[2][c] + red[3][c]);
}
inline int colsum_slices(int M, int N) {
    const int colblocks = (N + 63) / 64;
    int S = 2048 / colblocks;
    if (S > (M + 31) / 32) S = (M + 31) / 32;
    if (S > 256) S = 256;
    if (S < 1) S = 1;
    return S;
}

__global__ __launch_bounds__(256) void embed_gather_kernel(int rows, int E, const float* __restrict__ table, const int64_t* __restrict__ idx, float* __restrict__ out) {
    const int r = blockIdx.x;
    const int64_t id = idx[r];
    for (int e = threadIdx.x; e < E; e += 256) out[(size_t)r * E + e] = id < 0 ? 0.f : table[(size_t)id * E + e];
}
__global__ __launch_bounds__(256) void embed_gather_strided_kernel(int rows, int E, const float* __restrict__ table, const int64_t* __restrict__ idx,
                                                                   int istride, float* __restrict__ out, int ostride) {
    const int r = blockIdx.x;
    const int64_t id = idx[(size_t)r * istride];
    for (int e = threadIdx.x; e < E; e += 256) out[(size_t)r * ostride + e] = id < 0 ? 0.f : table[(size_t)id * E + e];
}
__global__ __launch_bounds__(256) void embed_scatter_det_kernel(int rows, int E, int V, const float* __restrict__ g, const int64_t* __restrict__ idx,
                                                                float* __restrict__ tg) {
    const int v = blockIdx.x * 4 + (threadIdx.x >> 6), lane = threadIdx.x & 63;
    if (v >= V) return;
    bool any = false;
    for (int r0 = 0; r0 < rows; r0 += 64) {
        const int r = r0 + lane;
        const bool hit = r < rows && idx[r] == (int64_t)v;
        unsigned long long ball = __ballot(hit);
        while (ball) {
            const int b = __ffsll((long long)ball) - 1;
            ball &= ball - 1;
            const float* src = g + (size_t)(r0 + b) * E;
            for (int e = lane; e < E; e += 64) tg[(size_t)v * E + e] += src[e];
            any = true;
        }
    }
    (void)any;
}
__global__ __launch_bounds__(256) void embed_scatter_kernel(int rows, int E, const float* __restrict__ g, const int64_t* __restrict__ idx, float* __restrict__ tg) {
    const int r = blockIdx.x;
    const int64_t id = idx[r];
    if (id < 0) return;
    for (int e = threadIdx.x; e < E; e += 256) atomicAdd(&tg[(size_t)id * E + e], g[(size_t)r * E + e]);
}

constexpr int SUMSQ_CHUNK = 256 * 4 * 8;
__global__ __launch_bounds__(256) void sumsq_kernel(size_t n, const float* __restrict__ x, double* __restrict__ partial, int vec) {
    __shared__ double red[4];
    const size_t base = (size_t)blockIdx.x * SUMSQ_CHUNK;
    float s = 0.f;
    if (vec && base + SUMSQ_CHUNK <= n) {
        const f32x4* x4 = reinterpret_cast<const f32x4*>(x + base);
#pragma unroll
        for (int i = 0; i < 8; ++i) { f32x4 v = x4[threadIdx.x + 256 * i]; s += v[0] * v[0] + v[1] * v[1] + v[2] * v[2] + v[3] * v[3]; }
    } else {
        for (size_t i = base + threadIdx.x; i < n && i < base + SUMSQ_CHUNK; i += 256) s += x[i] * x[i];
    }
    double d = wave_sum_d((double)s);
    if ((threadIdx.x & 63) == 0) red[threadIdx.x >> 6] = d;
    __syncthreads();
    if (threadIdx.x == 0) partial[blockIdx.x] = red[0] + red[1] + red[2] + red[3];
}

constexpr int GRAM_CHUNKS = 64;
struct GramJob { const float* gfac; size_t ldg; const float* afac; size_t lda; int rows, k; };
struct GramJobs { GramJob j[CAPHN_MAX_HEADS]; int n; };
__global__ __launch_bounds__(256) void rank_gram_kernel(int R, GramJobs jobs, double* __restrict__ ws) {
    __shared__ double red[4];
    const int pair = blockIdx.x, job = blockIdx.y >> 1, which = blockIdx.y & 1;
    const GramJob& J = jobs.j[job];
    const int r = pair / R, s = pair % R;
    const float* u = which ? J.afac + (size_t)r * J.lda : J.gfac + (size_t)r * J.ldg;
    const float* v = which ? J.afac + (size_t)s * J.lda : J.gfac + (size_t)s * J.ldg;
    const int n = which ? J.k : J.rows;
    const int per = (n + GRAM_CHUNKS - 1) / GRAM_CHUNKS;
    const int i0 = blockIdx.z * per, i1 = min(n, i0 + per);
    if (i0 >= i1) return;
    double acc = 0.0;
    for (int i = i0 + threadIdx.x; i < i1; i += 256) acc += (double)u[i] * (double)v[i];
    acc = wave_sum_d(acc);
    if ((threadIdx.x & 63) == 0) red[threadIdx.x >> 6] = acc;
    __syncthreads();
    if (threadIdx.x == 0) atomicAdd(&ws[((size_t)job * 2 + which) * R * R + pair], red[0] + red[1] + red[2] + red[3]);
}
__global__ void rank_gram_finish_kernel(int R, int njobs, const double* __restrict__ ws, double* acc) {
    if (threadIdx.x == 0 && blockIdx.x == 0) {
        double t = 0.0;
        for (int j = 0; j < njobs; ++j)
            for (int i = 0; i < R * R; ++i) t += ws[((size_t)j * 2) * R * R + i] * ws[((size_t)j * 2 + 1) * R * R + i];
        acc[0] += t;
    }
}
__global__ __launch_bounds__(256) void clip_coef_kernel(int nparts, const double* __restrict__ partial, const double* extra,
                                                        double max_norm, double scale, float* coef_out) {
    __shared__ double red[4];
// ... 602 lines not shown
    return caphn_launch_status();
}
extern "C" int caphn_add_dropout_f32(size_t n, const float* x, const float* branch, float p, unsigned long long seed,
                                     unsigned long long offset, float* out, caphn_stream_t stream) {
    if (n == 0) return CAPHN_OK;
    if (!x || !branch || !out || !(p >= 0.f) || !(p < 1.f)) return CAPHN_EINVAL;
    size_t blocks = (n + 255) / 256;
    if (blocks > 4096) blocks = 4096;
    hipLaunchKernelGGL(add_dropout_kernel, dim3((unsigned)blocks), dim3(256), 0, static_cast<hipStream_t>(stream), n, p, 1.0f / (1.0f - p), seed,
                       offset, x, branch, out);
    return caphn_launch_status();
}
extern "C" int caphn_scale_f32(size_t n, const float* x, const float* scale_dev, float* out, caphn_stream_t stream) {
    if (n == 0) return CAPHN_OK;
    if (!x || !scale_dev || !out) return CAPHN_EINVAL;
    size_t blocks = (n + 255) / 256;
    if (blocks > 4096) blocks = 4096;
    hipLaunchKernelGGL(scale_kernel, dim3((unsigned)blocks), dim3(256), 0, static_cast<hipStream_t>(stream), n, x, scale_dev, out);
    return caphn_launch_status();
}
extern "C" int caphn_lrelu_bwd_f32(size_t n, const float* dy, const float* post, float* dx, caphn_stream_t stream) {
    if (n == 0) return CAPHN_OK;
    if (!dy || !post || !dx) return CAPHN_EINVAL;
    size_t blocks = (n + 255) / 256;
    if (blocks > 1024) blocks = 1024;
    hipLaunchKernelGGL(lrelu_bwd_kernel, dim3((unsigned)blocks), dim3(256), 0, static_cast<hipStream_t>(stream), n, dy, post, dx);
    return caphn_launch_status();
}
extern "C" int caphn_axpy_f32(size_t n, float alpha, const float* x, float* y, caphn_stream_t stream) {
    if (n == 0) return CAPHN_OK;
    if (!x || !y) return CAPHN_EINVAL;
    size_t blocks = (n + 255) / 256;
    if (blocks > 2048) blocks = 2048;
    hipLaunchKernelGGL(axpy_kernel, dim3((unsigned)blocks), dim3(256), 0, static_cast<hipStream_t>(stream), n, alpha, x, y);
    return caphn_launch_status();
}
extern "C" int caphn_embedding_gather(int rows, int E, const float* table, const int64_t* idx, float* out, caphn_stream_t stream) {
    if (rows <= 0 || E <= 0 || !table || !idx || !out) return CAPHN_EINVAL;
    hipLaunchKernelGGL(embed_gather_kernel, dim3(rows), dim3(256), 0, static_cast<hipStream_t>(stream), rows, E, table, idx, out);
    return caphn_launch_status();
}
int caphn_embedding_gather_strided(int rows, int E, const float* table, const int64_t* idx, int istride, float* out, int ostride, hipStream_t s) {
    if (rows <= 0 || E <= 0 || !table || !idx || !out) return CAPHN_EINVAL;
    hipLaunchKernelGGL(embed_gather_strided_kernel, dim3(rows), dim3(256), 0, s, rows, E, table, idx, istride, out, ostride);
    return caphn_launch_status();
}
extern int g_tune_deterministic;
int g_det_vocab = 0;
extern "C" int caphn_embedding_scatter_add_v(int rows, int E, int V, const float* g, const int64_t* idx, float* table_grad,
                                             caphn_stream_t stream) {
    if (rows <= 0 || E <= 0 || V <= 0 || !g || !idx || !table_grad) return CAPHN_EINVAL;
    if (g_tune_deterministic && rows > 1) {
        hipLaunchKernelGGL(embed_scatter_det_kernel, dim3((V + 3) / 4), dim3(256), 0, static_cast<hipStream_t>(stream), rows, E,
                           V, g, idx, table_grad);
        return caphn_launch_status();
    }
    hipLaunchKernelGGL(embed_scatter_kernel, dim3(rows), dim3(256), 0, static_cast<hipStream_t>(stream), rows, E, g, idx, table_grad);
    return caphn_launch_status();
}
extern "C" int caphn_embedding_scatter_add(int rows, int E, const float* g, const int64_t* idx, float* table_grad, caphn_stream_t stream) {
    if (rows <= 0 || E <= 0 || !g || !idx || !table_grad) return CAPHN_EINVAL;
    if (g_tune_deterministic && g_det_vocab > 0 && rows > 1) return caphn_embedding_scatter_add_v(rows, E, g_det_vocab, g, idx, table_grad, stream);
    hipLaunchKernelGGL(embed_scatter_kernel, dim3(rows), dim3(256), 0, static_cast<hipStream_t>(stream), rows, E, g, idx, table_grad);
    return caphn_launch_status();
}

extern "C" int caphn_sumsq_blocks(size_t n) { return (int)((n + SUMSQ_CHUNK - 1) / SUMSQ_CHUNK); }
extern "C" int caphn_sumsq_f32(size_t n, const float* x, double* partial, caphn_stream_t stream) {
    if (n == 0 || !x || !partial) return CAPHN_EINVAL;
    const int nb = caphn_sumsq_blocks(n);
    hipLaunchKernelGGL(sumsq_kernel, dim3(nb), dim3(256), 0, static_cast<hipStream_t>(stream), n, x, partial, (int)caphn_aligned16(x));
    return caphn_launch_status();
}
extern "C" int caphn_rank_sumsq_f32(int R, int rows, int k, const float* gfac, size_t ldg, const float* afac, size_t lda,
                                    double* acc, double* ws, caphn_stream_t stream) {
    if (R <= 0 || R > RMAX || rows <= 0 || k <= 0 || !gfac || !afac || !acc || !ws) return CAPHN_EINVAL;
    hipStream_t s = static_cast<hipStream_t>(stream);
    GramJobs jobs; jobs.n = 1;
    jobs.j[0] = GramJob{gfac, ldg, afac, lda, rows, k};
    if (hipMemsetAsync(ws, 0, sizeof(double) * 2 * R * R, s) != hipSuccess) return CAPHN_ELAUNCH;
    hipLaunchKernelGGL(rank_gram_kernel, dim3(R * R, 2, GRAM_CHUNKS), dim3(256), 0, s, R, jobs, ws);
    hipLaunchKernelGGL(rank_gram_finish_kernel, dim3(1), dim3(64), 0, s, R, 1, ws, acc);
    return caphn_launch_status();
}
extern "C" int caphn_rank_sumsq_multi_f32(int R, int n, const int* rows, const int* k, const float* const* gfac, const size_t* ldg,
                                          const float* const* afac, const size_t* lda, double* acc, double* ws,
                                          caphn_stream_t stream) {
    if (R <= 0 || R > RMAX || n <= 0 || n > CAPHN_MAX_HEADS || !rows || !k || !gfac || !ldg || !afac || !lda || !acc || !ws)
        return CAPHN_EINVAL;
    hipStream_t s = static_cast<hipStream_t>(stream);
    GramJobs jobs; jobs.n = n;
    for (int i = 0; i < n; ++i) {
        if (rows[i] <= 0 || k[i] <= 0 || !gfac[i] || !afac[i]) return CAPHN_EINVAL;
        jobs.j[i] = GramJob{gfac[i], ldg[i], afac[i], lda[i], rows[i], k[i]};
    }
    if (hipMemsetAsync(ws, 0, sizeof(double) * 2 * R * R * n, s) != hipSuccess) return CAPHN_ELAUNCH;
    hipLaunchKernelGGL(rank_gram_kernel, dim3(R * R, 2 * n, GRAM_CHUNKS), dim3(256), 0, s, R, jobs, ws);
    hipLaunchKernelGGL(rank_gram_finish_kernel, dim3(1), dim3(64), 0, s, R, n, ws, acc);
    return caphn_launch_status();
}
extern "C" size_t caphn_grad_norm_workspace_bytes(size_t n, int R, int njobs) {
    if (R <= 0 || R > RMAX || njobs < 0 || njobs > CAPHN_MAX_HEADS) return 0;
    return sizeof(double) * ((size_t)caphn_sumsq_blocks(n) + (size_t)njobs * 2 * R * R * NORM_CHUNKS);
}
extern "C" int caphn_grad_norm_coef(size_t n, const float* x, int R, int njobs, const int* rows, const int* k,
                                    const float* const* gfac, const size_t* ldg, const float* const* afac, const size_t* lda,
                                    double max_norm, double scale, float* coef_out, void* ws, caphn_stream_t stream) {
    if (n == 0 || !x || R <= 0 || R > RMAX || njobs < 0 || njobs > CAPHN_MAX_HEADS || !coef_out || !ws) return CAPHN_EINVAL;
    GramJobs jobs; jobs.n = njobs;
    for (int i = 0; i < njobs; ++i) {
        if (!rows || !k || !gfac || !ldg || !afac || !lda || rows[i] <= 0 || k[i] <= 0 || !gfac[i] || !afac[i]) return CAPHN_EINVAL;
        jobs.j[i] = GramJob{gfac[i], ldg[i], afac[i], lda[i], rows[i], k[i]};
    }
    const int nb_s = caphn_sumsq_blocks(n);
    const unsigned nb = (unsigned)nb_s + (unsigned)(njobs * 2 * R * R * NORM_CHUNKS);
    hipStream_t s = static_cast<hipStream_t>(stream);
// ... 259 lines not shown
```

### hypernet-image-captioning_amd/csrc/recurrent_gru.hip

```cpp
#include "common.h"
#include "decoder_internal.h"

namespace {

constexpr int NT = 1024;
#ifdef CAPHN_REC_PROFILE
#define PSTAMP(i) do { if (prof_on) { unsigned long long _n = clock64(); pc[i] += _n - plast; plast = _n; } } while (0)
#define PDECL const bool prof_on = (b == 0 && tid == 0 && a.prof != nullptr); \
    unsigned long long pc[8] = {0, 0, 0, 0, 0, 0, 0, 0}, plast = prof_on ? clock64() : 0
#define PFLUSH do { if (prof_on) for (int i = 0; i < 8; ++i) a.prof[i] = pc[i]; } while (0)
#else
#define PSTAMP(i) do { } while (0)
#define PDECL do { } while (0)
#define PFLUSH do { } while (0)
#endif

__device__ __forceinline__ void copy_to_lds(float* dst, const float* __restrict__ src, int n, int vec, int tid) {
    if (vec) {
        const f32x4* s4 = reinterpret_cast<const f32x4*>(src);
        f32x4* d4 = reinterpret_cast<f32x4*>(dst);
        for (int i = tid; i < (n >> 2); i += NT) d4[i] = s4[i];
    } else {
        for (int i = tid; i < n; i += NT) dst[i] = src[i];
    }
// ... 18 lines not shown
            for (int c = s; c < K; c += 8) sum += row[c] * x_s[c];
        }
        sum += __shfl_xor(sum, 4, 64);
        sum += __shfl_xor(sum, 2, 64);
        sum += __shfl_xor(sum, 1, 64);
        if (s == 0) out_s[r] = sum + bias[r];
    }
}

constexpr int PGM = 10;
struct KG { int k, g, ng; };
__device__ __forceinline__ KG kg_map(int tid, int H) {
    KG m;
    m.ng = H >= NT ? 1 : NT / H;
    m.g = H >= NT ? 0 : tid / H;
    m.k = H >= NT ? tid : tid - m.g * H;
    if (m.g >= m.ng) { m.g = -1; }
    return m;
}

__device__ __forceinline__ void load_G_resident(float* G_s, const float* __restrict__ Gb, int P, int GH, int RGH,
                                                int vec, int tid) {
    if (RGH == GH) { copy_to_lds(G_s, Gb, P * GH, vec, tid); return; }
    if (vec) {
        const int r4 = RGH >> 2;
        for (int i = tid; i < P * r4; i += NT) {
            const int p = i / r4, c = i - p * r4;
            reinterpret_cast<f32x4*>(G_s + p * RGH)[c] = reinterpret_cast<const f32x4*>(Gb + (size_t)p * GH)[c];
        }
    } else {
        for (int i = tid; i < P * RGH; i += NT) { const int p = i / RGH, c = i - p * RGH; G_s[i] = Gb[(size_t)p * GH + c]; }
    }
}

template <bool LSTM>
__global__ __launch_bounds__(NT) void rec_attn_fwd_kernel(RecFwdArgs a) {
    constexpr int NG = LSTM ? 4 : 3;
    extern __shared__ __attribute__((aligned(16))) float lds[];
    const int b = blockIdx.x, tid = threadIdx.x, lane = tid & 63, wave = tid >> 6;
    const int P = a.P, H = a.H, GH = NG * a.H, T = a.T, RG = a.RG, RGH = a.RG * a.H;
    const int Ppad = (P + 63) & ~63;
    float* G_s = lds;
    float* h_s = G_s + P * RGH;
    float* uah_s = h_s + H;
    float* va_s = uah_s + H;
    float* c_s = va_s + H;
    float* gh_s = c_s + H;
    float* e_s = gh_s + GH;
    float* part_s = e_s + Ppad;

    const int sb = a.slab_div > 1 ? b / a.slab_div : b;
    const float* Gb = a.G + (size_t)sb * P * GH;
    load_G_resident(G_s, Gb, P, GH, RGH, a.vecS, tid);
    const int t0 = a.t0, t1 = a.t1 > 0 ? a.t1 : a.T;
    for (int k = tid; k < H; k += NT) {
        h_s[k] = t0 == 0 ? a.h0[(size_t)b * H + k] : (a.Hsrc ? a.Hsrc : a.Hs)[((size_t)b * T + t0 - 1) * H + k];
        va_s[k] = a.v_a[k];
        c_s[k] = LSTM ? (t0 == 0 ? a.c0[(size_t)b * H + k] : a.Cs[((size_t)b * T + t0 - 1) * H + k]) : 0.f;
    }
    const float bva = a.b_va[0];
    const float* Waf_b = a.Waf + (size_t)sb * P * H;
    const KG m = kg_map(tid, H);
    const int rotU = a.rotate ? (int)(((unsigned)b * 13u) % (unsigned)H) : 0;
    const int rotW = a.rotate ? (int)(((unsigned)b * 37u) % (unsigned)GH) : 0;
    constexpr int WP = 4, WK = 4;
    const bool waf_regs = (P <= WP * (NT / 64)) && (H <= WK * 64);
    float wreg[WP][WK];
#pragma unroll
    for (int i = 0; i < WP; ++i)
#pragma unroll
        for (int q = 0; q < WK; ++q) {
            const int p = wave + i * (NT / 64), k = lane + 64 * q;
            wreg[i][q] = (waf_regs && p < P && k < H) ? Waf_b[p * H + k] : 0.f;
        }
    __syncthreads();
    PDECL;

    for (int t = t0; t < t1; ++t) {
        const size_t bt = (size_t)b * T + t;
        matvec_rows(a.U_a, a.b_Ua, h_s, uah_s, H, H, a.vecW, tid, rotU);
        matvec_rows(a.W_hh, a.b_hh, h_s, gh_s, GH, H, a.vecW, tid, rotW);
        __syncthreads();
        PSTAMP(0);
        if (waf_regs) {
#pragma unroll
            for (int i = 0; i < WP; ++i) {
                const int p = wave + i * (NT / 64);
                if (p < P) {
                    float s = 0.f;
#pragma unroll
                    for (int q = 0; q < WK; ++q) {
                        const int k = lane + 64 * q;
                        if (k < H) s += va_s[k] * caphn_tanh(wreg[i][q] + uah_s[k]);
                    }
                    s = wave_sum(s);
                    if (lane == 0) e_s[p] = s + bva;
                }
            }
        } else {
            for (int p = wave; p < P; p += NT / 64) {
                float s = 0.f;
                for (int k = lane; k < H; k += 64) s += va_s[k] * caphn_tanh(Waf_b[p * H + k] + uah_s[k]);
                s = wave_sum(s);
                if (lane == 0) e_s[p] = s + bva;
            }
        }
        __syncthreads();
// ... 59 lines not shown
                a.gates[bt * GH + k] = r; a.gates[bt * GH + H + k] = z; a.gates[bt * GH + 2 * H + k] = n;
                a.hn[bt * H + k] = hnv;
            }
            if (a.drop_p > 0.f) hnew *= caphn_keep_scale(a.drop_seed, (unsigned long long)bt * H + k, a.drop_p, 1.0f / (1.0f - a.drop_p));
            a.Hprev[bt * H + k] = hp;
            a.Hs[bt * H + k] = hnew;
            a.uah[bt * H + k] = uah_s[k];
            h_s[k] = hnew;
        }
        __syncthreads();
        PSTAMP(4);
    }
    PFLUSH;
}

template <int CH>
__device__ __forceinline__ void matvec_t_accum(const float* __restrict__ W, const float* d_s, int rows, int H,
                                               int chunk, int slice, int nslices, float (&acc)[CH], int rot) {
    for (int j0 = slice; j0 < rows; j0 += nslices) {
        int j = j0 + rot;
        if (j >= rows) j -= rows;
        const float dj = d_s[j];
        const float* row = W + (size_t)j * H + chunk * CH;
        if (CH == 4) {
            f32x4 w = *reinterpret_cast<const f32x4*>(row);
            acc[0] += w[0] * dj; acc[1 % CH] += w[1] * dj; acc[2 % CH] += w[2] * dj; acc[3 % CH] += w[3] * dj;
        } else {
            acc[0] += row[0] * dj;
        }
    }
}

template <bool LSTM>
__global__ __launch_bounds__(NT) void rec_attn_bwd_kernel(RecBwdArgs a) {
    constexpr int NG = LSTM ? 4 : 3;
    extern __shared__ __attribute__((aligned(16))) float lds[];
    const int b = blockIdx.x, tid = threadIdx.x, lane = tid & 63, wave = tid >> 6;
    const int P = a.P, H = a.H, GH = NG * a.H, T = a.T, RG = a.RG, RGH = a.RG * a.H;
    const int Ppad = (P + 63) & ~63;
    float* G_s = lds;
    float* dh_s = G_s + P * RGH;
    float* dc_s = dh_s + H;
    float* duah_s = dc_s + H;
    float* uah_s = duah_s + H;
    float* va_s = uah_s + H;
    float* dgh_s = va_s + H;
    float* dgi_s = dgh_s + GH;
    float* dal_s = dgi_s + GH;
    float* al_s = dal_s + Ppad;
    float* part_s = al_s + Ppad;

    const float* Gb = a.G + (size_t)b * P * GH;
    load_G_resident(G_s, Gb, P, GH, RGH, a.vecS, tid);
    const int bt0 = a.t0, bt1 = a.t1 > 0 ? a.t1 : T;
    for (int k = tid; k < H; k += NT) {
        dh_s[k] = 0.f; va_s[k] = a.v_a[k];
        dc_s[k] = (LSTM && bt1 < T) ? a.dc0[(size_t)b * H + k] : 0.f;
    }
    const float* Waf_b = a.Waf + (size_t)b * P * H;
    const int CH = a.vecW ? 4 : 1;
    const int nch = (H + CH - 1) / CH;
    const int nch_eff = min(nch, NT);
    const int nslices = NT / nch_eff;
    const KG m = kg_map(tid, H);
    const int rotU = a.rotate ? (int)(((unsigned)b * 13u) % (unsigned)H) : 0;
    const int rotW = a.rotate ? (int)(((unsigned)b * 37u) % (unsigned)GH) : 0;
    __syncthreads();
    PDECL;
    const bool fuse = a.dWaf != nullptr && m.g >= 0;
    float dw[PGM];
#pragma unroll
    for (int i = 0; i < PGM; ++i) dw[i] = 0.f;
    float dva = 0.f, dbva = 0.f;

    for (int t = bt1 - 1; t >= bt0; --t) {
        const size_t bt = (size_t)b * T + t;
        for (int p = tid; p < P; p += NT) al_s[p] = a.alphas[bt * P + p];
        for (int k = tid; k < H; k += NT) {
            float dh = dh_s[k] + a.dHs[bt * H + k];
            if (a.drop_p > 0.f) dh *= caphn_keep_scale(a.drop_seed, (unsigned long long)bt * H + k, a.drop_p, 1.0f / (1.0f - a.drop_p));
            uah_s[k] = a.uah[bt * H + k];
            if (LSTM) {
                const float gi = a.gates[bt * GH + k], gf = a.gates[bt * GH + H + k], gg = a.gates[bt * GH + 2 * H + k];
                const float go = a.gates[bt * GH + (3 % NG) * H + k];
                const float cp = a.Cprev[bt * H + k];
                const float tc = caphn_tanh(a.Cs[bt * H + k]);
                const float d_o = dh * tc;
                const float dc = dc_s[k] + dh * go * (1.0f - tc * tc);
                const float dip = dc * gg * gi * (1.0f - gi);
                const float dfp = dc * cp * gf * (1.0f - gf);
                const float dgp = dc * gi * (1.0f - gg * gg);
                const float dop = d_o * go * (1.0f - go);
                dc_s[k] = dc * gf;
                dh_s[k] = 0.f;
                dgi_s[k] = dip; dgi_s[H + k] = dfp; dgi_s[2 * H + k] = dgp; dgi_s[(3 % NG) * H + k] = dop;
                dgh_s[k] = dip; dgh_s[H + k] = dfp; dgh_s[2 * H + k] = dgp; dgh_s[(3 % NG) * H + k] = dop;
                a.dgi[bt * GH + k] = dip; a.dgi[bt * GH + H + k] = dfp; a.dgi[bt * GH + 2 * H + k] = dgp;
                a.dgi[bt * GH + (3 % NG) * H + k] = dop;
            } else {
                const float r = a.gates[bt * GH + k], z = a.gates[bt * GH + H + k], n = a.gates[bt * GH + 2 * H + k];
                const float hnv = a.hn[bt * H + k], hp = a.Hprev[bt * H + k];
                const float dn = dh * (1.0f - z);
                const float dz = dh * (hp - n);
                const float dnp = dn * (1.0f - n * n);
                const float drp = dnp * hnv * r * (1.0f - r);
                const float dzp = dz * z * (1.0f - z);
                dh_s[k] = dh * z;
                dgi_s[k] = drp; dgi_s[H + k] = dzp; dgi_s[2 * H + k] = dnp;
                dgh_s[k] = drp; dgh_s[H + k] = dzp; dgh_s[2 * H + k] = dnp * r;
                a.dgi[bt * GH + k] = drp; a.dgi[bt * GH + H + k] = dzp; a.dgi[bt * GH + 2 * H + k] = dnp;
// ... 61 lines not shown
            a.duah[bt * H + k] = du;
        }
        __syncthreads();
        PSTAMP(4);
        {
            const int chunk = tid % nch_eff, slice = tid / nch_eff;
            if (slice < nslices) {
                for (int c = chunk; c < nch; c += nch_eff) {
                    if (CH == 4) {
                        float acc[4] = {0.f, 0.f, 0.f, 0.f};
                        matvec_t_accum<4>(a.W_hh, dgh_s, GH, H, c, slice, nslices, acc, rotW);
                        matvec_t_accum<4>(a.U_a, duah_s, H, H, c, slice, nslices, acc, rotU);
                        *reinterpret_cast<f32x4*>(part_s + slice * H + c * 4) = f32x4{acc[0], acc[1], acc[2], acc[3]};
                    } else {
                        float acc[1] = {0.f};
                        matvec_t_accum<1>(a.W_hh, dgh_s, GH, H, c, slice, nslices, acc, rotW);
                        matvec_t_accum<1>(a.U_a, duah_s, H, H, c, slice, nslices, acc, rotU);
                        part_s[slice * H + c] = acc[0];
                    }
                }
            }
        }
        __syncthreads();
        PSTAMP(5);
        for (int k = tid; k < H; k += NT) {
            float s = dh_s[k];
            for (int sl = 0; sl < nslices; ++sl) s += part_s[sl * H + k];
            dh_s[k] = s;
        }
        __syncthreads();
        PSTAMP(6);
    }
    PFLUSH;
    for (int k = tid; k < H; k += NT) {
        a.dh0[(size_t)b * H + k] = dh_s[k];
        if (LSTM) a.dc0[(size_t)b * H + k] = dc_s[k];
    }
    if (fuse) {
        const float vk = va_s[m.k];
#pragma unroll
        for (int i = 0; i < PGM; ++i) {
            const int p = m.g + i * m.ng;
            if (p < P) a.dWaf[((size_t)b * P + p) * H + m.k] = dw[i] * vk;
        }
        float* row = a.apart + ((size_t)b * m.ng + m.g) * (H + 1);
        row[m.k] = dva;
        if (m.k == 0) row[H] = dbva;
    }
}

__global__ void attn_param_grads_kernel(AttnGradArgs a) {
    const int b = blockIdx.x, pc = blockIdx.y;
    const int P = a.P, H = a.H, T = a.T;
    const int p0 = pc * a.pchunk, p1 = min(P, p0 + a.pchunk);
    const size_t blk = (size_t)b * gridDim.y + pc;
    for (int k = threadIdx.x; k < H; k += blockDim.x) {
        const float vk = a.v_a[k];
        float dv = 0.f;
        for (int p = p0; p < p1; ++p) {
            const float w = a.Waf[((size_t)b * P + p) * H + k];
            float s = 0.f;
#pragma unroll 4
            for (int t = 0; t < T; ++t) {
                const float de = a.de[((size_t)b * T + t) * P + p];
                const float tv = caphn_tanh(w + a.uah[((size_t)b * T + t) * H + k]);
                s += de * (1.0f - tv * tv);
                dv += de * tv;
            }
            a.dWaf[((size_t)b * P + p) * H + k] = s * vk;
        }
        a.part[blk * (H + 1) + k] = dv;
    }
    if (threadIdx.x == 0) {
        float s = 0.f;
        for (int p = p0; p < p1; ++p)
            for (int t = 0; t < T; ++t) s += a.de[((size_t)b * T + t) * P + p];
        a.part[blk * (H + 1) + H] = s;
    }
}

__global__ __launch_bounds__(256) void dmean_kernel(int H, int F, const float* __restrict__ dh0, const float* __restrict__ Wh,
                                                    const float* __restrict__ dc0, const float* __restrict__ Wc, float* __restrict__ out) {
    extern __shared__ float dv[];
    const int b = blockIdx.x;
    for (int j = threadIdx.x; j < H; j += 256) { dv[j] = dh0[(size_t)b * H + j]; dv[H + j] = dc0 ? dc0[(size_t)b * H + j] : 0.f; }
    __syncthreads();
    for (int k = threadIdx.x; k < F; k += 256) {
        float s0 = 0.f, s1 = 0.f;
        int j = 0;
        for (; j + 8 <= H; j += 8) {
            float w[8], c[8];
#pragma unroll
            for (int u = 0; u < 8; ++u) { w[u] = Wh[(size_t)(j + u) * F + k]; c[u] = dc0 ? Wc[(size_t)(j + u) * F + k] : 0.f; }
#pragma unroll
            for (int u = 0; u < 8; ++u) { s0 += dv[j + u] * w[u]; s1 += dv[H + j + u] * c[u]; }
        }
        for (; j < H; ++j) { s0 += dv[j] * Wh[(size_t)j * F + k]; if (dc0) s1 += dv[H + j] * Wc[(size_t)j * F + k]; }
        out[(size_t)b * F + k] = s0 + s1;
    }
}

__global__ void ctx_kernel(int P, int F, int T, const float* __restrict__ alphas, const float* __restrict__ f, float* __restrict__ ctx,
                           int ldc) {
    const int b = blockIdx.x, t = blockIdx.y;
    const float* al = alphas + ((size_t)b * T + t) * P;
    for (int k = threadIdx.x; k < F; k += blockDim.x) {
        float s = 0.f;
        int p = 0;
        for (; p + 8 <= P; p += 8) {
            float v[8];
#pragma unroll
            for (int u = 0; u < 8; ++u) v[u] = f[((size_t)b * P + p + u) * F + k];
#pragma unroll
            for (int u = 0; u < 8; ++u) s += al[p + u] * v[u];
        }
        for (; p < P; ++p) s += al[p] * f[((size_t)b * P + p) * F + k];
        ctx[((size_t)b * T + t) * ldc + k] = s;
    }
}
__global__ void df_kernel(int P, int F, int T, const float* __restrict__ alphas, const float* __restrict__ dctx,
                          const float* __restrict__ dmean, const float* __restrict__ dmean2, float* __restrict__ df) {
    const int b = blockIdx.x, p = blockIdx.y;
    const float invP = 1.0f / (float)P;
    for (int k = threadIdx.x; k < F; k += blockDim.x) {
        float s = (dmean2 ? dmean[(size_t)b * F + k] + dmean2[(size_t)b * F + k] : dmean[(size_t)b * F + k]) * invP;
        int t = 0;
        for (; t + 8 <= T; t += 8) {
            float a[8], v[8];
#pragma unroll
            for (int u = 0; u < 8; ++u) { a[u] = alphas[((size_t)b * T + t + u) * P + p]; v[u] = dctx[((size_t)b * T + t + u) * F + k]; }
#pragma unroll
            for (int u = 0; u < 8; ++u) s += a[u] * v[u];
        }
        for (; t < T; ++t) s += alphas[((size_t)b * T + t) * P + p] * dctx[((size_t)b * T + t) * F + k];
        df[((size_t)b * P + p) * F + k] = s;
    }
}
__global__ __launch_bounds__(1024) void init_state_kernel(int P, int F, int H, const float* __restrict__ f,
                                                          const float* __restrict__ Wh, const float* __restrict__ bh,
                                                          const float* __restrict__ Wc, const float* __restrict__ bc,
                                                          float* __restrict__ meanf, float* __restrict__ h0, float* __restrict__ c0) {
    extern __shared__ float sm[];
    const int b = blockIdx.x, tid = threadIdx.x, lane = tid & 63, wave = tid >> 6;
    const int Fp = (F + 255) & ~255;
    for (int k0 = 0; k0 < F; k0 += 256) {
        const int k = k0 + (tid & 255), pl = tid >> 8;
        float s = 0.f;
        if (k < F) for (int p = pl; p < P; p += 4) s += f[((size_t)b * P + p) * F + k];
        sm[pl * Fp + k0 + (tid & 255)] = s;
    }
    __syncthreads();
    const float invP = 1.0f / (float)P;
    for (int k = tid; k < F; k += 1024) {
        const float m = ((sm[k] + sm[Fp + k]) + (sm[2 * Fp + k] + sm[3 * Fp + k])) * invP;
        sm[4 * Fp + k] = m;
        meanf[(size_t)b * F + k] = m;
    }
    __syncthreads();
    const float* mean = sm + 4 * Fp;
    for (int j = wave; j < H; j += 16) {
        float sh = 0.f, sc = 0.f;
        for (int k = lane; k < F; k += 64) {
            const float m = mean[k];
            sh += Wh[(size_t)j * F + k] * m;
            if (Wc) sc += Wc[(size_t)j * F + k] * m;
        }
        sh = wave_sum(sh);
        if (Wc) sc = wave_sum(sc);
        if (lane == 0) {
            h0[(size_t)b * H + j] = sh + bh[j];
            if (Wc) c0[(size_t)b * H + j] = sc + bc[j];
        }
    }
}
__global__ void mean_p_kernel(int P, int F, const float* __restrict__ f, float* __restrict__ out) {
    const int b = blockIdx.x;
    const float invP = 1.0f / (float)P;
    for (int k = threadIdx.x; k < F; k += blockDim.x) {
        float s = 0.f;
        for (int p = 0; p < P; ++p) s += f[((size_t)b * P + p) * F + k];
        out[(size_t)b * F + k] = s * invP;
    }
}

constexpr size_t LDS_LIMIT = 160 * 1024;
bool g_attr_set[64];
int ensure_lds_attr() {
// ... 12 lines not shown

static int kg_groups(int H) { return H >= NT ? 1 : NT / H; }
size_t caphn_rec_fwd_lds_bytes(int P, int H, int NG, int RG) {
    const size_t Ppad = (P + 63) & ~63;
    return sizeof(float) * ((size_t)RG * P * H + 4 * (size_t)H + (size_t)NG * H + Ppad + (size_t)kg_groups(H) * NG * H);
}
size_t caphn_rec_bwd_lds_bytes(int P, int H, int NG, int RG) {
    const size_t Ppad = (P + 63) & ~63;
    const int CH = (H % 4 == 0) ? 4 : 1;
    const int nch = (H + CH - 1) / CH;
    const int nch_eff = nch < NT ? nch : NT;
    int nsl = NT / nch_eff;
    if (kg_groups(H) > nsl) nsl = kg_groups(H);
    const int nsl1 = NT / (H < NT ? H : NT);
    if (nsl1 > nsl) nsl = nsl1;
    return sizeof(float) * ((size_t)RG * P * H + 5 * (size_t)H + 2 * (size_t)NG * H + 2 * Ppad + (size_t)nsl * H);
}
int caphn_rec_resident_gates(int P, int H, int NG) {
    for (int rg = NG; rg >= 0; --rg)
        if (caphn_rec_fwd_lds_bytes(P, H, NG, rg) <= LDS_LIMIT && caphn_rec_bwd_lds_bytes(P, H, NG, rg) <= LDS_LIMIT) return rg;
    return -1;
}

int caphn_launch_rec_fwd(const RecFwdArgs& a, bool lstm, hipStream_t s) {
    const size_t lds = caphn_rec_fwd_lds_bytes(a.P, a.H, lstm ? 4 : 3, a.RG);
    if (lds > LDS_LIMIT) return CAPHN_ELIMIT;
    int rc = ensure_lds_attr(); if (rc) return rc;
    if (lstm) hipLaunchKernelGGL(rec_attn_fwd_kernel<true>, dim3(a.B), dim3(NT), lds, s, a);
    else hipLaunchKernelGGL(rec_attn_fwd_kernel<false>, dim3(a.B), dim3(NT), lds, s, a);
    return caphn_launch_status();
}
int caphn_rec_bwd_groups(int P, int H) {
    if (H > NT) return 0;
    const int ng = NT / H;
    return (P + ng - 1) / ng <= PGM ? ng : 0;
}
int caphn_launch_rec_bwd(const RecBwdArgs& a, bool lstm, hipStream_t s) {
    if (a.dWaf && (!a.apart || caphn_rec_bwd_groups(a.P, a.H) == 0)) return CAPHN_EINVAL;
    const size_t lds = caphn_rec_bwd_lds_bytes(a.P, a.H, lstm ? 4 : 3, a.RG);
    if (lds > LDS_LIMIT) return CAPHN_ELIMIT;
    int rc = ensure_lds_attr(); if (rc) return rc;
    if (lstm) hipLaunchKernelGGL(rec_attn_bwd_kernel<true>, dim3(a.B), dim3(NT), lds, s, a);
    else hipLaunchKernelGGL(rec_attn_bwd_kernel<false>, dim3(a.B), dim3(NT), lds, s, a);
    return caphn_launch_status();
}
int caphn_launch_attn_param_grads(const AttnGradArgs& a, int B, int npc, hipStream_t s) {
    hipLaunchKernelGGL(attn_param_grads_kernel, dim3(B, npc), dim3(a.H >= 192 ? 256 : 64), 0, s, a);
    return caphn_launch_status();
}
int caphn_launch_dmean(int B, int H, int F, const float* dh0, const float* Wh, const float* dc0, const float* Wc, float* out, hipStream_t s) {
    hipLaunchKernelGGL(dmean_kernel, dim3(B), dim3(256), sizeof(float) * 2 * H, s, H, F, dh0, Wh, dc0, Wc, out);
    return caphn_launch_status();
}
int caphn_launch_ctx(int B, int T, int P, int F, const float* alphas, const float* f, float* ctx, int ldc, hipStream_t s) {
    hipLaunchKernelGGL(ctx_kernel, dim3(B, T), dim3(F >= 192 ? 256 : 64), 0, s, P, F, T, alphas, f, ctx, ldc);
    return caphn_launch_status();
}
int caphn_launch_df(int B, int T, int P, int F, const float* alphas, const float* dctx, const float* dmean, float* df, hipStream_t s,
                    const float* dmean2) {
    hipLaunchKernelGGL(df_kernel, dim3(B, P), dim3(F >= 192 ? 256 : 64), 0, s, P, F, T, alphas, dctx, dmean, dmean2, df);
    return caphn_launch_status();
}
int caphn_launch_init_state(int B, int P, int F, int H, const float* f, const float* Wh, const float* bh, const float* Wc,
                            const float* bc, float* meanf, float* h0, float* c0, hipStream_t s) {
    const int Fp = (F + 255) & ~255;
    hipLaunchKernelGGL(init_state_kernel, dim3(B), dim3(1024), sizeof(float) * (4 * Fp + F), s, P, F, H, f, Wh, bh, Wc, bc, meanf, h0, c0);
    return caphn_launch_status();
}
int caphn_launch_mean_p(int B, int P, int F, const float* f, float* out, hipStream_t s) {
    hipLaunchKernelGGL(mean_p_kernel, dim3(B), dim3(F >= 192 ? 256 : 64), 0, s, P, F, f, out);
    return caphn_launch_status();
}
```

### hypernet-image-captioning_amd/csrc/recurrent_pair.hip

```cpp
#include "common.h"
#include "decoder_internal.h"
#include <atomic>

namespace {

constexpr int NT = 512;
#ifdef CAPHN_REC_PROFILE
#define PSTAMP(i) do { if (prof_on) { unsigned long long _n = clock64(); pc[i] += _n - plast; plast = _n; } } while (0)
#define PDECL const bool prof_on = (w == 0 && tid == 0 && a.prof != nullptr); \
    unsigned long long pc[8] = {0, 0, 0, 0, 0, 0, 0, 0}, plast = prof_on ? clock64() : 0
#define PFLUSH do { if (prof_on) for (int i = 0; i < 8; ++i) a.prof[i] = pc[i]; } while (0)
#else
#define PSTAMP(i) do { } while (0)
#define PDECL do { } while (0)
#define PFLUSH do { } while (0)
#endif

typedef unsigned long long u64;

__device__ int d_pair_opts = 0;
__device__ __forceinline__ void xsend(u64* slot, float v, unsigned tag, bool near = false) {
    const u64 bits = ((u64)tag << 32) | (u64)__float_as_uint(v);
    if (near) __hip_atomic_store(slot, bits, __ATOMIC_RELAXED, __HIP_MEMORY_SCOPE_WORKGROUP);
    else __hip_atomic_store(slot, bits, __ATOMIC_RELAXED, __HIP_MEMORY_SCOPE_AGENT);
// ... 195 lines not shown
        }
    }
}

template <bool LSTM, int CM>
__global__ __launch_bounds__(NT) void rec_pair_fwd_kernel(RecFwdArgs a) {
    constexpr bool CACHED = CM != 0;
    constexpr int NG = LSTM ? 4 : 3;
    extern __shared__ __attribute__((aligned(16))) float lds[];
    const int w = blockIdx.x, tid = threadIdx.x, lane = tid & 63, wave = tid >> 6;
    const int b = (w & 7) + 8 * (w >> 4), hh = (w >> 3) & 1;
    if (b >= a.B) return;
    const int P = a.P, H = a.H, GH = NG * a.H, RG = a.RG;
    const int Ppad = (P + 63) & ~63;
    const HalfK hk = half_of(H, hh);
    const int k0 = hk.k0, nk = hk.nk, nkm = half_a(H);
    const float* WPh = a.WP + (size_t)hh * (NG + 1) * nkm * a.wp_pitch;
    float* G_s = lds;
    float* h_s = G_s + (size_t)P * RG * nkm;
    float* va_s = h_s + ((H + 3) & ~3);
    float* c_s = va_s + nkm;
    float* out_s = c_s + nkm;
    float* uah_s = out_s;
    float* gh_s = out_s + nk;
    float* e_s = out_s + (NG + 1) * nkm;
    float* part_s = e_s + Ppad;
    float* bias_s = part_s + (size_t)kg_map(0, H - nkm > 0 ? H - nkm : 1).ng * NG * nkm;
    float* Waf_s = bias_s + (size_t)(NG + 1) * nkm;
    float* Wc_s = Waf_s + (a.waf_lds ? (size_t)P * nkm : 0);

    u64* xmine = a.xch + (size_t)w * xch_stride(P, H);
    u64* xpart = a.xch + (size_t)(w ^ 8) * xch_stride(P, H);
    u64* xh_mine = xmine; u64* xe_mine = xmine + nkm;
    u64* xh_part = xpart; u64* xe_part = xpart + nkm;
    const unsigned ep = a.epoch << 16;
    const XCtl xc{a.err, a.xlimit};
    const bool mute = d_skip_xrecv == 2 && hh == 1;
    const bool near = partner_is_near(xmine + xch_ctl(P, H), xpart + xch_ctl(P, H), ep | 0xFFFFu, a.err, a.xlimit, tid, reinterpret_cast<int*>(e_s));

    const float* Gb = a.G + (size_t)b * P * GH;
    const int vecS = a.vecS && (nk % 4 == 0) && (k0 % 4 == 0);
    if (vecS) {
        const int n4 = nk >> 2;
        for (int i = tid; i < P * RG * n4; i += NT) {
            const int c = i % n4, pq = i / n4, q = pq % RG, p = pq / RG;
            reinterpret_cast<f32x4*>(G_s + (size_t)pq * nk)[c] = reinterpret_cast<const f32x4*>(Gb + (size_t)p * GH + q * H + k0)[c];
        }
    } else {
        for (int i = tid; i < P * RG * nk; i += NT) {
            const int kk = i % nk, pq = i / nk, q = pq % RG, p = pq / RG;
            G_s[(size_t)pq * nk + kk] = Gb[(size_t)p * GH + q * H + k0 + kk];
        }
    }
    const int t0 = a.t0, t1 = a.t1 > 0 ? a.t1 : a.T, T = a.T;
    for (int k = tid; k < H; k += NT)
        h_s[k] = t0 == 0 ? a.h0[(size_t)b * H + k] : (a.Hsrc ? a.Hsrc : a.Hs)[((size_t)b * T + t0 - 1) * H + k];
    for (int kk = tid; kk < nk; kk += NT) {
        va_s[kk] = a.v_a[k0 + kk];
        c_s[kk] = LSTM ? (t0 == 0 ? a.c0[(size_t)b * H + k0 + kk] : a.Cs[((size_t)b * T + t0 - 1) * H + k0 + kk]) : 0.f;
    }
    const float bva = hh == 0 ? a.b_va[0] : 0.f;
    const float* Waf_b = a.Waf + (size_t)b * P * H;
    const KG m = kg_map(tid, nk);
    constexpr int WP = 8, WK = 2;
    const bool waf_regs = a.waf_lds && (P <= WP * (NT / 64)) && (nk <= WK * 64);
    for (int r = tid; r < (NG + 1) * nk; r += NT) {
        const int q = r / nk, kk = r - q * nk;
        bias_s[r] = q == 0 ? a.b_Ua[k0 + kk] : a.b_hh[(q - 1) * H + k0 + kk];
    }
    if (a.waf_lds)
        for (int i = tid; i < P * nk; i += NT) { const int p = i / nk, kk = i - p * nk; Waf_s[(size_t)p * nkm + kk] = Waf_b[p * H + k0 + kk]; }
    const int NR = (NG + 1) * nk;
    const int grp = tid >> 3, s8 = tid & 7;
    const int vecW = (H % 4) == 0;
    constexpr int WRC = CM == 2 ? FULL_RC : CACHED ? 2 : 1;
    constexpr bool cached = CACHED;
    const int NL = cached ? a.wc_rows : 0;
    f32x4 wc[WRC][JM];
    if (cached) {
        const int n4 = H >> 2;
#pragma unroll
        for (int i = 0; i < WRC; ++i) {
            const f32x4* row = reinterpret_cast<const f32x4*>(pair_row(WPh, a.wp_pitch, min((NT / 8) * i + grp, NR - 1)));
#pragma unroll
            for (int j = 0; j < JM; ++j) wc[i][j] = row[s8 + 8 * j];
        }
        for (int idx = tid; idx < NL * n4; idx += NT) {
            const int slot = idx / n4, c = idx - slot * n4;
            const int r = min((NT / 8) * (WRC + slot / (NT / 8)) + slot % (NT / 8), NR - 1);
            reinterpret_cast<f32x4*>(Wc_s)[idx] = reinterpret_cast<const f32x4*>(pair_row(WPh, a.wp_pitch, r))[c];
        }
    }
    __syncthreads();
    PDECL;

    for (int t = t0; t < t1; ++t) {
        const size_t bt = (size_t)b * T + t;
        float xgq[NG];
#pragma unroll
        for (int q = 0; q < NG; ++q) xgq[q] = tid < nk ? a.Xg[bt * GH + q * H + k0 + tid] : 0.f;
        if (t > t0) {
            for (int j = tid; j < hk.nkp; j += NT) h_s[hk.k0p + j] = xrecv(xh_part + j, xtag(ep, t - 1, 1), xc);
            __syncthreads();
        }
        PSTAMP(1);
        if constexpr (cached) pair_matvec_cached<WRC, CM != 2>(WPh, a.wp_pitch, bias_s, h_s, out_s, H, NR, grp, s8, wc, Wc_s, NL);
        else pair_matvec(WPh, a.wp_pitch, bias_s, h_s, out_s, H, NR, vecW, grp, s8);
// ... 146 lines not shown

template <bool LSTM, int TCR>
__global__ __launch_bounds__(NT) void rec_pair_bwd_kernel(RecBwdArgs a) {
    constexpr int NG = LSTM ? 4 : 3;
    constexpr int PGM = 10;
    constexpr int TU = 8;
    extern __shared__ __attribute__((aligned(16))) float lds[];
    const int w = blockIdx.x, tid = threadIdx.x, lane = tid & 63, wave = tid >> 6;
    const int b = (w & 7) + 8 * (w >> 4), hh = (w >> 3) & 1;
    if (b >= a.B) return;
    const int P = a.P, H = a.H, GH = NG * a.H, T = a.T, RG = a.RG;
    const int Ppad = (P + 63) & ~63;
    const HalfK hk = half_of(H, hh);
    const int k0 = hk.k0, nk = hk.nk, nkm = half_a(H);
    const int H4 = (H + 3) & ~3;
    const float* WPh = a.WP + (size_t)hh * (NG + 1) * nkm * a.wp_pitch;
    float* G_s = lds;
    float* dh_s = G_s + (size_t)P * RG * nkm;
    float* dc_s = dh_s + nkm;
    float* uah_s = dc_s + nkm;
    float* va_s = uah_s + nkm;
    float* duah_s = va_s + nkm;
    float* dgh_s = duah_s + nk;
    float* dgi_s = duah_s + (NG + 1) * nkm;
    float* dal_s = dgi_s + NG * nkm;
    float* al_s = dal_s + Ppad;
    float* dhp_s = al_s + Ppad;
    float* part_s = dhp_s + H4;
    float* Wc_s = part_s + (size_t)a.part_rows * H4;

    u64* xmine = a.xch + (size_t)w * xch_stride(P, H);
    u64* xpart = a.xch + (size_t)(w ^ 8) * xch_stride(P, H);
    u64* xh_mine = xmine; u64* xe_mine = xmine + nkm;
    u64* xh_part = xpart; u64* xe_part = xpart + nkm;
    const unsigned ep = a.epoch << 16;
    const XCtl xc{a.err, a.xlimit};
    const bool mute = d_skip_xrecv == 2 && hh == 1;
    const bool near = partner_is_near(xmine + xch_ctl(P, H), xpart + xch_ctl(P, H), ep | 0xFFFFu, a.err, a.xlimit, tid, reinterpret_cast<int*>(dal_s));

    const float* Gb = a.G + (size_t)b * P * GH;
    const int vecS = a.vecS && (nk % 4 == 0) && (k0 % 4 == 0);
    if (vecS) {
        const int n4 = nk >> 2;
        for (int i = tid; i < P * RG * n4; i += NT) {
            const int c = i % n4, pq = i / n4, q = pq % RG, p = pq / RG;
            reinterpret_cast<f32x4*>(G_s + (size_t)pq * nk)[c] = reinterpret_cast<const f32x4*>(Gb + (size_t)p * GH + q * H + k0)[c];
        }
    } else {
        for (int i = tid; i < P * RG * nk; i += NT) {
            const int kk = i % nk, pq = i / nk, q = pq % RG, p = pq / RG;
            G_s[(size_t)pq * nk + kk] = Gb[(size_t)p * GH + q * H + k0 + kk];
        }
    }
    const int bt0 = a.t0, bt1 = a.t1 > 0 ? a.t1 : T;
    for (int kk = tid; kk < nk; kk += NT) {
        dh_s[kk] = 0.f; va_s[kk] = a.v_a[k0 + kk];
        dc_s[kk] = (LSTM && bt1 < T) ? a.dc0[(size_t)b * H + k0 + kk] : 0.f;
    }
    const float* Waf_b = a.Waf + (size_t)b * P * H;
    const int CH = (H % 4) == 0 ? 4 : 1;
    const KG m = kg_map(tid, nk);
    const int NR = (NG + 1) * nk;
    __syncthreads();
    const bool fuse = a.dWaf != nullptr && m.g >= 0;
    float dw[PGM];
#pragma unroll
    for (int i = 0; i < PGM; ++i) dw[i] = 0.f;
    float wafr[PGM];
#pragma unroll
    for (int i = 0; i < PGM; ++i) { const int p = m.g + i * m.ng; wafr[i] = (fuse && p < P) ? Waf_b[p * H + k0 + m.k] : 0.f; }
    float dva = 0.f, dbva = 0.f;
    PDECL;

    f32x4 wreg[TCR > 0 ? TCR : 1];
    const int tc_nch = (H + 3) / 4, tc_nsl = NT / (tc_nch < NT ? tc_nch : NT);
    const int tc_chunk = tid % tc_nch, tc_slice = tid / tc_nch;
    if constexpr (TCR > 0) {
#pragma unroll
        for (int u = 0; u < TCR; ++u) {
            const int r = a.wc_rows + tc_slice + u * tc_nsl;
            wreg[u] = (tc_slice < tc_nsl && r < NR) ? *reinterpret_cast<const f32x4*>(WPh + (size_t)r * a.wp_pitch + tc_chunk * 4)
                                                     : f32x4{0.f, 0.f, 0.f, 0.f};
        }
    }
    const float* dvec_s = duah_s;
    auto tmatvec = [&](int cb, int ce) {
        if constexpr (TCR > 0) {
            if (tc_slice < tc_nsl) {
                float acc[4] = {0.f, 0.f, 0.f, 0.f};
                for (int r = tc_slice; r < a.wc_rows;) {
                    f32x4 wv[4]; float dj[4];
#pragma unroll
                    for (int u = 0; u < 4; ++u) {
                        wv[u] = *reinterpret_cast<const f32x4*>(Wc_s + (size_t)r * H + tc_chunk * 4);
                        dj[u] = dvec_s[r];
                        r += tc_nsl;
                    }
#pragma unroll
                    for (int u = 0; u < 4; ++u) { acc[0] += wv[u][0] * dj[u]; acc[1] += wv[u][1] * dj[u]; acc[2] += wv[u][2] * dj[u]; acc[3] += wv[u][3] * dj[u]; }
                }
#pragma unroll
                for (int u0 = 0; u0 < TCR; u0 += 8) {
                    float dj[8];
#pragma unroll
                    for (int u = 0; u < 8; ++u) { const int r = a.wc_rows + tc_slice + (u0 + u) * tc_nsl; dj[u] = (u0 + u < TCR && r < NR) ? dvec_s[r] : 0.f; }
#pragma unroll
                    for (int u = 0; u < 8; ++u)
                        if (u0 + u < TCR) { const f32x4 w = wreg[u0 + u]; acc[0] += w[0] * dj[u]; acc[1] += w[1] * dj[u]; acc[2] += w[2] * dj[u]; acc[3] += w[3] * dj[u]; }
                }
                *reinterpret_cast<f32x4*>(part_s + (size_t)tc_slice * H4 + tc_chunk * 4) = f32x4{acc[0], acc[1], acc[2], acc[3]};
// ... 33 lines not shown
                while (r < NR) {
                    const float* rp[TU]; float dj[TU];
#pragma unroll
                    for (int u = 0; u < TU; ++u) {
                        const bool ok = r < NR;
                        rp[u] = col + (size_t)(ok ? r : 0) * a.wp_pitch;
                        dj[u] = ok ? dvec_s[r] : 0.f;
                        r += nsl;
                    }
                    if (CH == 4) {
                        f32x4 wv[TU];
#pragma unroll
                        for (int u = 0; u < TU; ++u) wv[u] = *reinterpret_cast<const f32x4*>(rp[u]);
#pragma unroll
                        for (int u = 0; u < TU; ++u) { acc[0] += wv[u][0] * dj[u]; acc[1] += wv[u][1] * dj[u]; acc[2] += wv[u][2] * dj[u]; acc[3] += wv[u][3] * dj[u]; }
                    } else {
#pragma unroll
                        for (int u = 0; u < TU; ++u) acc[0] += rp[u][0] * dj[u];
                    }
                }
                if (CH == 4) *reinterpret_cast<f32x4*>(part_s + (size_t)slice * H4 + c * 4) = f32x4{acc[0], acc[1], acc[2], acc[3]};
                else part_s[(size_t)slice * H4 + c] = acc[0];
            }
        }
        __syncthreads();
        for (int j = tid; j < ncol; j += NT) {
            float sum = 0.f;
            for (int sl = 0; sl < nsl; ++sl) sum += part_s[(size_t)sl * H4 + j];
            dhp_s[cb + j] = sum;
        }
        __syncthreads();
    };
    if (a.wc_rows > 0) {
        const int n4 = H >> 2;
        for (int idx = tid; idx < a.wc_rows * n4; idx += NT) {
            const int r = idx / n4, c = idx - r * n4;
            reinterpret_cast<f32x4*>(Wc_s)[idx] = reinterpret_cast<const f32x4*>(WPh + (size_t)r * a.wp_pitch)[c];
        }
        __syncthreads();
    }
    const bool pfk = nk <= NT && P <= NT;
    float pf[8] = {0.f, 0.f, 0.f, 0.f, 0.f, 0.f, 0.f, 0.f}, pfa = 0.f;
    auto prefetch = [&](int t) {
        const size_t bt = (size_t)b * T + t;
        if (tid < P) pfa = a.alphas[bt * P + tid];
        if (tid < nk) {
            const int k = k0 + tid;
            pf[0] = a.dHs[bt * H + k]; pf[1] = a.uah[bt * H + k];
            pf[2] = a.gates[bt * GH + k]; pf[3] = a.gates[bt * GH + H + k]; pf[4] = a.gates[bt * GH + 2 * H + k];
            if (LSTM) { pf[5] = a.gates[bt * GH + (3 % NG) * H + k]; pf[6] = a.Cprev[bt * H + k]; pf[7] = a.Cs[bt * H + k]; }
            else { pf[5] = a.hn[bt * H + k]; pf[6] = a.Hprev[bt * H + k]; }
        }
    };
    if (pfk) prefetch(bt1 - 1);

    for (int t = bt1 - 1; t >= bt0; --t) {
        const size_t bt = (size_t)b * T + t;
        if (pfk) { if (tid < P) al_s[tid] = pfa; }
        else for (int p = tid; p < P; p += NT) al_s[p] = a.alphas[bt * P + p];
        for (int kk = tid; kk < nk; kk += NT) {
            const int k = k0 + kk;
            float dh = dh_s[kk] + (pfk ? pf[0] : a.dHs[bt * H + k]);
            if (a.drop_p > 0.f) dh *= caphn_keep_scale(a.drop_seed, (unsigned long long)bt * H + k, a.drop_p, 1.0f / (1.0f - a.drop_p));
            uah_s[kk] = pfk ? pf[1] : a.uah[bt * H + k];
            if (LSTM) {
                const float gi = pfk ? pf[2] : a.gates[bt * GH + k], gf = pfk ? pf[3] : a.gates[bt * GH + H + k];
                const float gg = pfk ? pf[4] : a.gates[bt * GH + 2 * H + k];
                const float go = pfk ? pf[5] : a.gates[bt * GH + (3 % NG) * H + k];
                const float cp = pfk ? pf[6] : a.Cprev[bt * H + k];
                const float tc = caphn_tanh(pfk ? pf[7] : a.Cs[bt * H + k]);
                const float d_o = dh * tc;
                const float dc = dc_s[kk] + dh * go * (1.0f - tc * tc);
                const float dip = dc * gg * gi * (1.0f - gi);
                const float dfp = dc * cp * gf * (1.0f - gf);
                const float dgp = dc * gi * (1.0f - gg * gg);
                const float dop = d_o * go * (1.0f - go);
                dc_s[kk] = dc * gf;
                dh_s[kk] = 0.f;
                dgi_s[kk] = dip; dgi_s[nk + kk] = dfp; dgi_s[2 * nk + kk] = dgp; dgi_s[(3 % NG) * nk + kk] = dop;
                dgh_s[kk] = dip; dgh_s[nk + kk] = dfp; dgh_s[2 * nk + kk] = dgp; dgh_s[(3 % NG) * nk + kk] = dop;
                a.dgi[bt * GH + k] = dip; a.dgi[bt * GH + H + k] = dfp; a.dgi[bt * GH + 2 * H + k] = dgp;
                a.dgi[bt * GH + (3 % NG) * H + k] = dop;
            } else {
                const float r = pfk ? pf[2] : a.gates[bt * GH + k], z = pfk ? pf[3] : a.gates[bt * GH + H + k];
                const float n = pfk ? pf[4] : a.gates[bt * GH + 2 * H + k];
                const float hnv = pfk ? pf[5] : a.hn[bt * H + k], hp = pfk ? pf[6] : a.Hprev[bt * H + k];
                const float dn = dh * (1.0f - z);
                const float dz = dh * (hp - n);
                const float dnp = dn * (1.0f - n * n);
                const float drp = dnp * hnv * r * (1.0f - r);
                const float dzp = dz * z * (1.0f - z);
                dh_s[kk] = dh * z;
                dgi_s[kk] = drp; dgi_s[nk + kk] = dzp; dgi_s[2 * nk + kk] = dnp;
                dgh_s[kk] = drp; dgh_s[nk + kk] = dzp; dgh_s[2 * nk + kk] = dnp * r;
                a.dgi[bt * GH + k] = drp; a.dgi[bt * GH + H + k] = dzp; a.dgi[bt * GH + 2 * H + k] = dnp;
                a.dgh[bt * GH + k] = drp; a.dgh[bt * GH + H + k] = dzp; a.dgh[bt * GH + 2 * H + k] = dnp * r;
            }
        }
        if (pfk && t > bt0) prefetch(t - 1);
        __syncthreads();
        PSTAMP(0);
        if (RG == NG && P <= 8 * (NT / 64) && nk <= 128) {
            float sp[8], dg[NG][2];
#pragma unroll
            for (int q = 0; q < NG; ++q)
#pragma unroll
                for (int c = 0; c < 2; ++c) { const int kk = lane + 64 * c; dg[q][c] = kk < nk ? dgi_s[q * nk + kk] : 0.f; }
// ... 357 lines not shown
```

### include/caphn.h

```cpp
#ifndef CAPHN_H
#define CAPHN_H
#include <stdint.h>
#include <stddef.h>

#ifdef __cplusplus
extern "C" {
#endif

typedef void* caphn_stream_t;

#define CAPHN_OK 0
#define CAPHN_EINVAL (-1)
#define CAPHN_ELAUNCH (-2)
#define CAPHN_ELIMIT (-3)
#define CAPHN_ETIMEOUT (-4)

int caphn_abi_version(void);
int caphn_device_error(int clear);
int caphn_device_arch(char* buf, int buflen);

#define CAPHN_GEMM_BIAS 1
#define CAPHN_GEMM_RELU 2
#define CAPHN_GEMM_ACCUM 4
#define CAPHN_GEMM_MASK 8
// ... 64 lines not shown
    int raw_features;
    int row_subset;
    int grads_zeroed;
    int precomputed;
    int layers;
    float dropout_p;
    unsigned long long dropout_seed;
    int logits_ld;
} caphn_decoder_dims;

#define CAPHN_MAX_DEC_LAYERS 4
typedef struct caphn_decoder_params {
    const float* fc0_w; const float* fc0_b;
    const float* fc2_w; const float* fc2_b;
    const float* embed_w;
    const float* out_w; const float* out_b;
    const float* Wa_w; const float* Wa_b;
    const float* Ua_w; const float* Ua_b;
    const float* va_w; const float* va_b;
    const float* inith_w; const float* inith_b;
    const float* w_ih; const float* w_hh;
    const float* b_ih; const float* b_hh;
    const float* initc_w; const float* initc_b;
    const float* lw_ih[CAPHN_MAX_DEC_LAYERS - 1]; const float* lw_hh[CAPHN_MAX_DEC_LAYERS - 1];
    const float* lb_ih[CAPHN_MAX_DEC_LAYERS - 1]; const float* lb_hh[CAPHN_MAX_DEC_LAYERS - 1];
} caphn_decoder_params;

typedef struct caphn_decoder_grads {
    float* fc0_w; float* fc0_b; float* fc2_w; float* fc2_b;
    float* embed_w;
    float* out_w; float* out_b;
    float* Wa_w; float* Wa_b; float* Ua_w; float* Ua_b; float* va_w; float* va_b;
    float* inith_w; float* inith_b;
    float* w_ih; float* w_hh; float* b_ih; float* b_hh;
    float* initc_w; float* initc_b;
    float* lw_ih[CAPHN_MAX_DEC_LAYERS - 1]; float* lw_hh[CAPHN_MAX_DEC_LAYERS - 1];
    float* lb_ih[CAPHN_MAX_DEC_LAYERS - 1]; float* lb_hh[CAPHN_MAX_DEC_LAYERS - 1];
} caphn_decoder_grads;

size_t caphn_decoder_workspace_bytes(const caphn_decoder_dims* d);
int caphn_decoder_forward(const caphn_decoder_dims* d, const caphn_decoder_params* p,
                          const float* features, const int64_t* captions,
                          float* logits, float* alphas, void* ws, caphn_stream_t stream);
int caphn_decoder_precompute(const caphn_decoder_dims* d, const caphn_decoder_params* p, const float* features,
                             const int64_t* captions , void* ws, caphn_stream_t stream);
int caphn_decoder_inputs(const caphn_decoder_dims* d, const caphn_decoder_params* p, const int64_t* captions, void* ws,
                         caphn_stream_t stream);
int caphn_decoder_lookup(const caphn_decoder_dims* d, const caphn_decoder_params* p, const int64_t* captions, void* ws,
                         caphn_stream_t stream);
typedef struct caphn_pair_pack { float* wp; int H, HA, pitch, hrows; } caphn_pair_pack;
int caphn_decoder_pair_prep(const caphn_decoder_dims* d, const caphn_decoder_params* p, void* ws, caphn_stream_t stream);
int caphn_decoder_pair_pack_desc(const caphn_decoder_dims* d, void* ws, caphn_pair_pack* out);
const int* caphn_decoder_rowcount_ptr(const caphn_decoder_dims* d, void* ws);
int caphn_decoder_prepare_rows(const caphn_decoder_dims* d, const int64_t* targets, int64_t ignore_index,
                               void* ws, caphn_stream_t stream);
unsigned long long* caphn_decoder_profile_ptr(const caphn_decoder_dims* d, void* ws);
int caphn_decoder_forward_sampled(const caphn_decoder_dims* d, const caphn_decoder_params* p,
                                  const float* features, const int64_t* captions,
                                  const unsigned char* use_sampling,
                                  float* logits, float* alphas, void* ws, caphn_stream_t stream);
int caphn_decoder_forward_sampled_train(const caphn_decoder_dims* d, const caphn_decoder_params* p,
                                        const float* features, const int64_t* captions,
                                        const unsigned char* use_sampling,
                                        float* logits, float* alphas, void* ws, caphn_stream_t stream);
int caphn_decoder_backward(const caphn_decoder_dims* d, const caphn_decoder_params* p,
                           const float* features, const int64_t* captions,
                           float* dlogits, const float* dalphas,
                           const caphn_decoder_grads* g, void* ws, caphn_stream_t stream);

int caphn_decoder_hyper_backward(const caphn_decoder_dims* d, const caphn_decoder_params* p,
                                 const float* features, const int64_t* captions,
                                 float* dlogits, const float* dalphas,
                                 const caphn_decoder_grads* g, void* ws,
                                 const caphn_hyper_desc* hd, const float* acts, const caphn_hyper_grads* hg, void* hyper_ws,
                                 caphn_stream_t stream);

#define CAPHN_MS_DTHETA 0
#define CAPHN_MS_VOCAB 1
#define CAPHN_MS_EMBED 2
#define CAPHN_MS_HYPER 3
#define CAPHN_MS_COUNT 4
int caphn_decoder_backward_milestone(int which, caphn_stream_t waiter);

typedef struct {
    int n_images, beam, max_steps;
    int zero_pad_rule, lookup_first;
    int64_t first_token, end_token;
} caphn_search_cfg;
size_t caphn_decoder_search_workspace_bytes(const caphn_decoder_dims* d, const caphn_search_cfg* c);
int caphn_decoder_search_begin(const caphn_decoder_dims* d, const caphn_decoder_params* p, const caphn_search_cfg* c,
                               const float* features, void* ws, void* search_ws, caphn_stream_t stream);
int caphn_decoder_search_steps(const caphn_decoder_dims* d, const caphn_decoder_params* p, const caphn_search_cfg* c,
                               int step0, int nsteps, float* alphas, void* ws, void* search_ws, caphn_stream_t stream);
int caphn_decoder_search_result(const caphn_decoder_dims* d, const caphn_search_cfg* c, int steps_done, void* ws, void* search_ws,
                                int64_t* seqs, int* lengths, float* scores, int* finished, int* n_active,
                                caphn_stream_t stream);

#define CAPHN_MAX_LAYERS 4
typedef struct caphn_plain_dims { int B, T, E, H, V, L, cell; } caphn_plain_dims;
typedef struct caphn_plain_params {
    const float* embed_w; const float* out_w; const float* out_b;
    const float* w_ih[CAPHN_MAX_LAYERS]; const float* w_hh[CAPHN_MAX_LAYERS];
    const float* b_ih[CAPHN_MAX_LAYERS]; const float* b_hh[CAPHN_MAX_LAYERS];
} caphn_plain_params;
typedef struct caphn_plain_grads {
    float* embed_w; float* out_w; float* out_b;
// ... 117 lines not shown
```

Measured before the change: 80280 images/s.

## Skip padded trailing timesteps per caption in recurrence and backward kernels

Computes each caption's live length (last non-ignored target) and a compacted step map, then truncates the forward/backward recurrent loops, context, df, attention-param-grad and embedding-scatter kernels to live steps, and routes weight-gradient GEMMs through the step map. Padding steps past a caption's end are skipped instead of computed, with their gradient buffers zeroed. This lowers recurrent and GEMM work in proportion to padding, at the cost of an extra pass in the row-map kernel and mapped GEMM indirection. It depends on padded steps not affecting the loss, which holds when targets are ignored after the end.

```diff
diff --git a/hypernet-image-captioning_amd/caphn/_lib.py b/hypernet-image-captioning_amd/caphn/_lib.py
--- a/hypernet-image-captioning_amd/caphn/_lib.py
+++ b/hypernet-image-captioning_amd/caphn/_lib.py
@@ -158,6 +158,7 @@
     "caphn_cross_entropy_finish": (C.c_int, [C.c_int, c_fp, c_fp, c_fp, c_fp]),
     "caphn_decoder_profile_ptr": (C.c_void_p, [C.POINTER(DecoderDims), c_fp]),
     "caphn_decoder_rowcount_ptr": (C.c_void_p, [C.POINTER(DecoderDims), c_fp]),
+    "caphn_decoder_stepmap_ptr": (C.c_void_p, [C.POINTER(DecoderDims), c_fp, C.POINTER(C.c_void_p)]),
     "caphn_cross_entropy_fwd_bwd": (C.c_int, [C.c_int, C.c_int, c_fp, c_fp, C.c_int64, c_fp, c_fp, C.c_int, c_fp, c_fp]),
     "caphn_embedding_gather": (C.c_int, [C.c_int, C.c_int, c_fp, c_fp, c_fp, c_fp]),
     "caphn_embedding_scatter_add": (C.c_int, [C.c_int, C.c_int, c_fp, c_fp, c_fp, c_fp]),
diff --git a/hypernet-image-captioning_amd/caphn/ops.py b/hypernet-image-captioning_amd/caphn/ops.py
--- a/hypernet-image-captioning_amd/caphn/ops.py
+++ b/hypernet-image-captioning_amd/caphn/ops.py
@@ -598,6 +598,13 @@
     return int(L.load().caphn_decoder_rowcount_ptr(C.byref(cd), C.c_void_p(ws.data_ptr())) or 0)
 
 
+def decoder_stepmap_ptrs(dims: DecDims, ws: torch.Tensor) -> Tuple[int, int]:
+    cd = dims.c()
+    nl = C.c_void_p()
+    sm = L.load().caphn_decoder_stepmap_ptr(C.byref(cd), C.c_void_p(ws.data_ptr()), C.byref(nl))
+    return int(sm or 0), int(nl.value or 0)
+
+
 def embedding_gather(table: torch.Tensor, idx: torch.Tensor) -> torch.Tensor:
     lib = L.load()
     rows, E = idx.numel(), table.shape[1]
diff --git a/hypernet-image-captioning_amd/csrc/decoder.hip b/hypernet-image-captioning_amd/csrc/decoder.hip
--- a/hypernet-image-captioning_amd/csrc/decoder.hip
+++ b/hypernet-image-captioning_amd/csrc/decoder.hip
@@ -14,6 +14,7 @@
 int g_tune_chain_main = 0;
 int g_tune_hops = 0;
 int g_tune_fork = 4;
+int g_tune_live_steps = 1;
 int g_tune_join_chain = 0;
 int g_tune_sk_dhs = 0, g_tune_sk_vocab_w = 0;
 #define RUN(x) do { int _rc = (x); if (_rc != CAPHN_OK) return _rc; } while (0)
@@ -136,6 +137,7 @@
 struct Ws {
     size_t Y1, f, meanf, h0, c0, Waf, G, Xe, Xg, Hs, Hprev, gates, hn, Cs, Cprev, uah, alphas, idx;
     size_t dHs, dgi, dgh, duah, de, dh0, dc0, ctx, dctx, dXe, dWaf, dmeanf, df, dY1, apart, vtmp, colws, colws_s[3], prof, rowmap;
+    size_t stepmap, nlive;
     size_t xch, xch_floats;
     size_t wp;
     size_t H0s, dH0, h0L, dcarry, tgi, tgh, tmpA, tmpB;
@@ -148,6 +150,10 @@
 inline bool use_pair(const caphn_decoder_dims* d) {
     const int NG = d->cell == CAPHN_CELL_LSTM ? 4 : 3;
     return g_tune_rec_pair && d->T > 1 && d->layers <= 1 && caphn_rec_pair_resident_gates(d->P, d->H, NG) >= 0;
+}
+
+inline bool use_live(const caphn_decoder_dims* d, const void* alphas_or_dalphas) {
+    return g_tune_live_steps && d->row_subset && d->layers <= 1 && alphas_or_dalphas == nullptr;
 }
 
 inline size_t up4(size_t v) { return (v + 3) & ~(size_t)3; }
@@ -191,6 +197,8 @@
     }
     w.prof = take(64);
     w.rowmap = take(B * T + 4);
+    w.stepmap = take(B * T + 4);
+    w.nlive = take(B);
     w.xch_floats = caphn_rec_pair_xch_bytes((int)B, (int)P, (int)H) / sizeof(float);
     w.xch = take(2 * w.xch_floats);
     o = (o + 31) & ~(size_t)31;
@@ -211,15 +219,23 @@
     return w;
 }
 
-__global__ __launch_bounds__(1024) void valid_rows_kernel(int n, const int64_t* __restrict__ tgt, int64_t ignore, int* __restrict__ map) {
+__global__ __launch_bounds__(1024) void valid_rows_kernel(int n, const int64_t* __restrict__ tgt, int64_t ignore, int* __restrict__ map,
+                                                          int B, int T, int* __restrict__ nlive, int* __restrict__ smap) {
     __shared__ int wsum[16];
     __shared__ int base_s;
     const int tid = threadIdx.x, lane = tid & 63, wave = tid >> 6;
+    for (int b = tid; b < B; b += 1024) {
+        int t = T;
+        while (t > 0 && tgt[(size_t)b * T + t - 1] == ignore) --t;
+        nlive[b] = t;
+    }
     if (tid == 0) base_s = 0;
     __syncthreads();
+    for (int pass = 0; pass < 2; ++pass) {
+    if (pass == 1) { map = smap; if (tid == 0) base_s = 0; __syncthreads(); }
     for (int c0 = 0; c0 < n; c0 += 1024) {
         const int i = c0 + tid;
-        const int v = (i < n && tgt[i] != ignore) ? 1 : 0;
+        const int v = i >= n ? 0 : pass == 0 ? (tgt[i] != ignore ? 1 : 0) : (i % T < nlive[i / T] ? 1 : 0);
         const unsigned long long ball = __ballot(v);
         const int before = __popcll(ball & ((1ull << lane) - 1ull));
         if (lane == 0) wsum[wave] = __popcll(ball);
@@ -233,6 +249,8 @@
         __syncthreads();
     }
     if (tid == 0) map[0] = base_s;
+    __syncthreads();
+    }
 }
 
 __global__ void copy2_kernel(const float* __restrict__ src, int n, float* __restrict__ a, float* __restrict__ b) {
@@ -419,6 +437,13 @@
     return reinterpret_cast<const int*>(static_cast<float*>(ws_) + layout(d).rowmap);
 }
 
+extern "C" const int* caphn_decoder_stepmap_ptr(const caphn_decoder_dims* d, void* ws_, const int** nlive_out) {
+    if (!dims_ok(d) || !ws_) return nullptr;
+    const Ws w = layout(d);
+    if (nlive_out) *nlive_out = reinterpret_cast<const int*>(static_cast<float*>(ws_) + w.nlive);
+    return reinterpret_cast<const int*>(static_cast<float*>(ws_) + w.stepmap);
+}
+
 extern "C" unsigned long long* caphn_decoder_profile_ptr(const caphn_decoder_dims* d, void* ws_) {
     if (!dims_ok(d) || !ws_) return nullptr;
     return reinterpret_cast<unsigned long long*>(static_cast<float*>(ws_) + layout(d).prof);
@@ -428,8 +453,10 @@
                                           void* ws_, caphn_stream_t stream) {
     if (!dims_ok(d) || !targets || !ws_) return CAPHN_EINVAL;
     const Ws w = layout(d);
+    float* ws = static_cast<float*>(ws_);
     hipLaunchKernelGGL(valid_rows_kernel, dim3(1), dim3(1024), 0, static_cast<hipStream_t>(stream), d->B * d->T, targets,
-                       ignore_index, reinterpret_cast<int*>(static_cast<float*>(ws_) + w.rowmap));
+                       ignore_index, reinterpret_cast<int*>(ws + w.rowmap), d->B, d->T, reinterpret_cast<int*>(ws + w.nlive),
+                       reinterpret_cast<int*>(ws + w.stepmap));
     return caphn_launch_status();
 }
 
@@ -524,6 +551,7 @@
     if (pc & 16)
         RUN(sdw->await(Side::D_PRE_ALL, s));
 
+    const int* nlive = use_live(d, alphas) ? reinterpret_cast<const int*>(ws + w.nlive) : nullptr;
     RecFwdArgs a;
     a.B = B; a.T = T; a.P = P; a.H = H; a.RG = RG;
     a.Waf = ws + w.Waf; a.G = ws + w.G; a.Xg = ws + w.Xg; a.h0 = ws + w.h0; a.c0 = ws + w.c0;
@@ -534,6 +562,7 @@
     a.vecS = (H % 4 == 0) && caphn_aligned16(ws);
     a.prof = reinterpret_cast<unsigned long long*>(ws + w.prof);
     a.rotate = g_tune_rec_rotate;
+    a.nlive = nlive;
     a.drop_p = d->dropout_p; a.drop_seed = d->dropout_seed;
     if (pair) {
         a.xch = reinterpret_cast<unsigned long long*>(ws + w.xch);
@@ -560,7 +589,7 @@
                               reinterpret_cast<const int*>(ws + w.rowmap) + 4, reinterpret_cast<const int*>(ws + w.rowmap), 1, s));
     else
         RUN(caphn_gemm_f32(0, 1, BT, V, H, ws + w.Hs, H, p->out_w, H, logits, LV, p->out_b, nullptr, 0, CAPHN_GEMM_BIAS, 1, s));
-    if (pc & 32) RUN(caphn_launch_ctx(B, T, P, F, ws + w.alphas, f, ws + w.ctx, EF, s));
+    if (pc & 32) RUN(caphn_launch_ctx(B, T, P, F, ws + w.alphas, f, ws + w.ctx, EF, s, nlive));
     if (alphas)
         if (hipMemcpyAsync(alphas, ws + w.alphas, sizeof(float) * (size_t)BT * P, hipMemcpyDeviceToDevice, s) != hipSuccess)
             return CAPHN_ELAUNCH;
@@ -623,6 +652,8 @@
     void* cw0 = ws + w.colws_s[0]; void* cw1 = ws + w.colws_s[1]; void* cw2 = ws + w.colws_s[2];
 
     const int* rmap = d->row_subset ? reinterpret_cast<const int*>(ws + w.rowmap) : nullptr;
+    const int* nlive = use_live(d, dalphas) ? reinterpret_cast<const int*>(ws + w.nlive) : nullptr;
+    const int* smap = nlive ? reinterpret_cast<const int*>(ws + w.stepmap) : nullptr;
     const int LV = d->logits_ld > 0 ? d->logits_ld : V;
     const int fork_mode = g_tune_fork == 4 ? (pair ? 2 : 1) : g_tune_fork;
     const bool late = fork_mode != 2;
@@ -645,7 +676,7 @@
     if (!late && !wg_first) {
         if (!(d->precomputed & 32) && sd.s(0) != s && sd.s(2) != s) {
             RUN(sd.fork_many({0, 2}));
-            RUN(caphn_launch_ctx(B, T, P, F, ws + w.alphas, f, ws + w.ctx, EF, sd.s(2)));
+            RUN(caphn_launch_ctx(B, T, P, F, ws + w.alphas, f, ws + w.ctx, EF, sd.s(2), nlive));
             RUN(sd.record(5, sd.s(2)));
             ctx_side = true;
         } else
@@ -665,6 +696,7 @@
     a.vecS = (H % 4 == 0) && caphn_aligned16(ws);
     a.prof = reinterpret_cast<unsigned long long*>(ws + w.prof) + 8;
     a.rotate = g_tune_rec_rotate;
+    a.nlive = nlive;
     a.drop_p = d->dropout_p; a.drop_seed = d->dropout_seed;
     const int ang = w.L1 > 0 ? 0 : pair ? caphn_rec_pair_bwd_groups(P, H) : caphn_rec_bwd_groups(P, H);
     if (ang > 0) { a.dWaf = ws + w.dWaf; a.apart = ws + w.apart; }
@@ -696,16 +728,18 @@
         RUN(sd.milestone(CAPHN_MS_VOCAB, b0));
     }
     if (ctx_side) RUN(sd.wait(5, sT));
-    else if (!(d->precomputed & 32)) RUN(caphn_launch_ctx(B, T, P, F, ws + w.alphas, f, ws + w.ctx, EF, sT));
-    if (lstm) RUN(gemm_auto(1, 0, GH, EF, BT, dgi, GH, ws + w.Xe, EF, g->w_ih, EF, nullptr, 0, sT, nullptr, 0, gz));
-    else RUN(wgrad_bias(GH, EF, BT, dgi, GH, ws + w.Xe, EF, g->w_ih, EF, g->b_ih, nullptr, cw1, sT, gz));
-    RUN(wgrad_bias(GH, H, BT, dgh, GH, ws + w.Hprev, H, g->w_hh, H, g->b_hh, nullptr, cw2, b2, gz));
+    else if (!(d->precomputed & 32)) RUN(caphn_launch_ctx(B, T, P, F, ws + w.alphas, f, ws + w.ctx, EF, sT, nlive));
+    if (lstm) RUN(gemm_auto(1, 0, GH, EF, BT, dgi, GH, ws + w.Xe, EF, g->w_ih, EF, nullptr, 0, sT, smap, 2, gz));
+    else RUN(wgrad_bias(GH, EF, BT, dgi, GH, ws + w.Xe, EF, g->w_ih, EF, g->b_ih, smap, cw1, sT, gz));
+    RUN(wgrad_bias(GH, H, BT, dgh, GH, ws + w.Hprev, H, g->w_hh, H, g->b_hh, smap, cw2, b2, gz));
     if (lstm) RUN(caphn_colsum_f32(BT, GH, dgi, GH, g->b_ih, cw2, b2));
     RUN(sd.record(3, b2));
     hipStream_t se = late ? b2 : b0;
-    RUN(caphn_gemm_f32(0, 0, BT, E, GH, dgi, GH, p->w_ih, EF, ws + w.dXe, E, nullptr, nullptr, 0, 0, 1, se));
+    if (smap) RUN(caphn_gemm_mapped(0, 0, BT, E, GH, dgi, GH, p->w_ih, EF, ws + w.dXe, E, nullptr, 0, 1, smap + 4, smap, 1, se));
+    else RUN(caphn_gemm_f32(0, 0, BT, E, GH, dgi, GH, p->w_ih, EF, ws + w.dXe, E, nullptr, nullptr, 0, 0, 1, se));
     if (!gz) RUN(caphn_zero_f32(g->embed_w, (size_t)V * E, se));
-    RUN(caphn_embedding_scatter_add_v(BT, E, V, ws + w.dXe, idx, g->embed_w, se));
+    if (smap) RUN(caphn_embedding_scatter_add_live(BT, E, V, ws + w.dXe, idx, g->embed_w, nlive, T, se));
+    else RUN(caphn_embedding_scatter_add_v(BT, E, V, ws + w.dXe, idx, g->embed_w, se));
     RUN(sd.milestone(CAPHN_MS_EMBED, se));
     RUN(sd.wait(3, sT));
     RUN(sd.milestone(CAPHN_MS_DTHETA, sT));
@@ -714,6 +748,8 @@
     }
     if (!hold_big) RUN(sd.milestone(CAPHN_MS_HYPER, sT));
     if (!raw) {
+        if (smap) RUN(caphn_gemm_mapped(0, 0, BT, F, GH, dgi, GH, p->w_ih + E, EF, ws + w.dctx, F, nullptr, 0, 1, smap + 4, smap, 1, sF));
+        else
         RUN(caphn_gemm_f32(0, 0, BT, F, GH, dgi, GH, p->w_ih + E, EF, ws + w.dctx, F, nullptr, nullptr, 0, 0, 1, sF));
         if (!pair)
             RUN(caphn_launch_dmean(B, H, F, ws + w.dh0, p->inith_w, lstm ? ws + w.dc0 : nullptr, lstm ? p->initc_w : nullptr,
@@ -722,10 +758,10 @@
     AttnGradArgs ag;
     ag.T = T; ag.P = P; ag.H = H; ag.pchunk = w.pchunk;
     ag.Waf = ws + w.Waf; ag.uah = ws + w.uah; ag.de = ws + w.de; ag.v_a = p->va_w;
-    ag.dWaf = ws + w.dWaf; ag.part = ws + w.apart;
+    ag.dWaf = ws + w.dWaf; ag.part = ws + w.apart; ag.nlive = nlive;
     if (ang == 0) RUN(caphn_launch_attn_param_grads(ag, B, w.npc, sF));
     RUN(sd.record(2, sF));
-    RUN(wgrad_bias(H, H, BT, ws + w.duah, H, ws + w.Hprev, H, g->Ua_w, H, g->Ua_b, nullptr, cws, b0, gz));
+    RUN(wgrad_bias(H, H, BT, ws + w.duah, H, ws + w.Hprev, H, g->Ua_w, H, g->Ua_b, smap, cws, b0, gz));
     for (int l = 0; l < w.L1; ++l) {
         const int BS = B * (T + 1), G3 = 3 * H;
         RUN(wgrad_bias(G3, H, BS, ws + w.Ldgi[l], G3, ws + w.Lin[l], H, g->lw_ih[l], H, g->lb_ih[l], nullptr, cws, b0, gz));
@@ -734,7 +770,7 @@
     RUN(wgrad_bias(H, F, B, ws + w.dh0, H, ws + w.meanf, F, g->inith_w, F, g->inith_b, nullptr, cws, b0, gz));
     if (lstm) RUN(wgrad_bias(H, F, B, ws + w.dc0, H, ws + w.meanf, F, g->initc_w, F, g->initc_b, nullptr, cws, b0, gz));
     if (!raw) {
-        RUN(caphn_launch_df(B, T, P, F, ws + w.alphas, ws + w.dctx, ws + w.dmeanf, ws + w.df, sF, pair ? ws + w.dmeanf + (size_t)B * F : nullptr));
+        RUN(caphn_launch_df(B, T, P, F, ws + w.alphas, ws + w.dctx, ws + w.dmeanf, ws + w.df, sF, pair ? ws + w.dmeanf + (size_t)B * F : nullptr, nlive));
         RUN(caphn_gemm_f32(0, 0, BP, F, H, ws + w.dWaf, H, p->Wa_w, F, ws + w.df, F, nullptr, nullptr, 0, CAPHN_GEMM_ACCUM, 1, sF));
         RUN(sd.record(4, sF));
         if (hold_big) {
diff --git a/hypernet-image-captioning_amd/csrc/decoder_internal.h b/hypernet-image-captioning_amd/csrc/decoder_internal.h
--- a/hypernet-image-captioning_amd/csrc/decoder_internal.h
+++ b/hypernet-image-captioning_amd/csrc/decoder_internal.h
@@ -29,6 +29,7 @@
     int wc_rows = 0;
     unsigned epoch = 0; int* err = nullptr; long long xlimit = 0;
     const float* Hsrc = nullptr;
+    const int* nlive = nullptr;
 };
 struct RecBwdArgs {
     int B, T, P, H;
@@ -55,12 +56,14 @@
     const float* inith_w = nullptr; const float* initc_w = nullptr; float* dmean_part = nullptr; int F = 0;
     int part_rows = 0, wc_rows = 0;
     int t0 = 0, t1 = 0;
+    const int* nlive = nullptr;
 };
 struct AttnGradArgs {
     int T, P, H, pchunk;
     const float* Waf; const float* uah; const float* de; const float* v_a;
     float* dWaf;
     float* part;
+    const int* nlive = nullptr;
 };
 
 struct LayerFwdArgs {
@@ -100,9 +103,13 @@
 int caphn_launch_rec_pair_bwd(const RecBwdArgs& a, bool lstm, hipStream_t s);
 int caphn_rec_bwd_groups(int P, int H);
 int caphn_launch_attn_param_grads(const AttnGradArgs& a, int B, int npc, hipStream_t s);
-int caphn_launch_ctx(int B, int T, int P, int F, const float* alphas, const float* f, float* ctx, int ldc, hipStream_t s);
+int caphn_launch_ctx(int B, int T, int P, int F, const float* alphas, const float* f, float* ctx, int ldc, hipStream_t s,
+                     const int* nlive = nullptr);
 int caphn_launch_df(int B, int T, int P, int F, const float* alphas, const float* dctx, const float* dmean, float* df, hipStream_t s,
-                    const float* dmean2 = nullptr);
+                    const float* dmean2 = nullptr,
+                    const int* nlive = nullptr);
+int caphn_embedding_scatter_add_live(int rows, int E, int V, const float* g, const int64_t* idx, float* table_grad, const int* nlive, int T,
+                                     hipStream_t s);
 int caphn_launch_dmean(int B, int H, int F, const float* dh0, const float* Wh, const float* dc0, const float* Wc, float* out, hipStream_t s);
 int caphn_launch_init_state(int B, int P, int F, int H, const float* f, const float* Wh, const float* bh, const float* Wc,
                             const float* bc, float* meanf, float* h0, float* c0, hipStream_t s);
diff --git a/hypernet-image-captioning_amd/csrc/hyper.hip b/hypernet-image-captioning_amd/csrc/hyper.hip
--- a/hypernet-image-captioning_amd/csrc/hyper.hip
+++ b/hypernet-image-captioning_amd/csrc/hyper.hip
@@ -851,6 +851,7 @@
 extern int g_tune_adam_dense_cap;
 extern int g_tune_sk_dhs, g_tune_sk_vocab_w;
 extern int g_tune_join_chain;
+extern int g_tune_live_steps;
 extern int g_tune_gemm_kres;
 extern int g_tune_gemm_waves;
 extern int g_tune_hops;
@@ -882,6 +883,7 @@
     if (key == 27) { g_tune_hyper_tail = value != 0; return CAPHN_OK; }
     if (key == 28) { g_tune_acts_fused = value != 0; return CAPHN_OK; }
     if (key == 36) { g_tune_gemm_kres = value != 0; return CAPHN_OK; }
+    if (key == 37) { g_tune_live_steps = value != 0; return CAPHN_OK; }
     if (key == 35) { g_tune_join_chain = value != 0; return CAPHN_OK; }
     if (key == 33) { if (value < 0 || value > 64) return CAPHN_EINVAL; g_tune_sk_dhs = value; return CAPHN_OK; }
     if (key == 34) { if (value < 0 || value > 64) return CAPHN_EINVAL; g_tune_sk_vocab_w = value; return CAPHN_OK; }
diff --git a/hypernet-image-captioning_amd/csrc/misc.hip b/hypernet-image-captioning_amd/csrc/misc.hip
--- a/hypernet-image-captioning_amd/csrc/misc.hip
+++ b/hypernet-image-captioning_amd/csrc/misc.hip
@@ -219,13 +219,13 @@
     for (int e = threadIdx.x; e < E; e += 256) out[(size_t)r * ostride + e] = id < 0 ? 0.f : table[(size_t)id * E + e];
 }
 __global__ __launch_bounds__(256) void embed_scatter_det_kernel(int rows, int E, int V, const float* __restrict__ g, const int64_t* __restrict__ idx,
-                                                                float* __restrict__ tg) {
+                                                                float* __restrict__ tg, const int* __restrict__ nlive, int T) {
     const int v = blockIdx.x * 4 + (threadIdx.x >> 6), lane = threadIdx.x & 63;
     if (v >= V) return;
     bool any = false;
     for (int r0 = 0; r0 < rows; r0 += 64) {
         const int r = r0 + lane;
-        const bool hit = r < rows && idx[r] == (int64_t)v;
+        const bool hit = r < rows && idx[r] == (int64_t)v && (!nlive || r % T < nlive[r / T]);
         unsigned long long ball = __ballot(hit);
         while (ball) {
             const int b = __ffsll((long long)ball) - 1;
@@ -237,10 +237,12 @@
     }
     (void)any;
 }
-__global__ __launch_bounds__(256) void embed_scatter_kernel(int rows, int E, const float* __restrict__ g, const int64_t* __restrict__ idx, float* __restrict__ tg) {
+__global__ __launch_bounds__(256) void embed_scatter_kernel(int rows, int E, const float* __restrict__ g, const int64_t* __restrict__ idx, float* __restrict__ tg,
+                                                            const int* __restrict__ nlive, int T) {
     const int r = blockIdx.x;
     const int64_t id = idx[r];
     if (id < 0) return;
+    if (nlive && r % T >= nlive[r / T]) return;
     for (int e = threadIdx.x; e < E; e += 256) atomicAdd(&tg[(size_t)id * E + e], g[(size_t)r * E + e]);
 }
 
@@ -949,16 +951,25 @@
     if (rows <= 0 || E <= 0 || V <= 0 || !g || !idx || !table_grad) return CAPHN_EINVAL;
     if (g_tune_deterministic && rows > 1) {
         hipLaunchKernelGGL(embed_scatter_det_kernel, dim3((V + 3) / 4), dim3(256), 0, static_cast<hipStream_t>(stream), rows, E,
-                           V, g, idx, table_grad);
+                           V, g, idx, table_grad, nullptr, 1);
         return caphn_launch_status();
     }
-    hipLaunchKernelGGL(embed_scatter_kernel, dim3(rows), dim3(256), 0, static_cast<hipStream_t>(stream), rows, E, g, idx, table_grad);
+    hipLaunchKernelGGL(embed_scatter_kernel, dim3(rows), dim3(256), 0, static_cast<hipStream_t>(stream), rows, E, g, idx, table_grad, nullptr, 1);
+    return caphn_launch_status();
+}
+int caphn_embedding_scatter_add_live(int rows, int E, int V, const float* g, const int64_t* idx, float* table_grad, const int* nlive, int T,
+                                     hipStream_t s) {
+    if (rows <= 0 || E <= 0 || V <= 0 || T <= 0 || !g || !idx || !table_grad || !nlive) return CAPHN_EINVAL;
+    if (g_tune_deterministic && rows > 1)
+        hipLaunchKernelGGL(embed_scatter_det_kernel, dim3((V + 3) / 4), dim3(256), 0, s, rows, E, V, g, idx, table_grad, nlive, T);
+    else
+        hipLaunchKernelGGL(embed_scatter_kernel, dim3(rows), dim3(256), 0, s, rows, E, g, idx, table_grad, nlive, T);
     return caphn_launch_status();
 }
 extern "C" int caphn_embedding_scatter_add(int rows, int E, const float* g, const int64_t* idx, float* table_grad, caphn_stream_t stream) {
     if (rows <= 0 || E <= 0 || !g || !idx || !table_grad) return CAPHN_EINVAL;
     if (g_tune_deterministic && g_det_vocab > 0 && rows > 1) return caphn_embedding_scatter_add_v(rows, E, g_det_vocab, g, idx, table_grad, stream);
-    hipLaunchKernelGGL(embed_scatter_kernel, dim3(rows), dim3(256), 0, static_cast<hipStream_t>(stream), rows, E, g, idx, table_grad);
+    hipLaunchKernelGGL(embed_scatter_kernel, dim3(rows), dim3(256), 0, static_cast<hipStream_t>(stream), rows, E, g, idx, table_grad, nullptr, 1);
     return caphn_launch_status();
 }
 
diff --git a/hypernet-image-captioning_amd/csrc/recurrent_gru.hip b/hypernet-image-captioning_amd/csrc/recurrent_gru.hip
--- a/hypernet-image-captioning_amd/csrc/recurrent_gru.hip
+++ b/hypernet-image-captioning_amd/csrc/recurrent_gru.hip
@@ -94,7 +94,7 @@
     const int sb = a.slab_div > 1 ? b / a.slab_div : b;
     const float* Gb = a.G + (size_t)sb * P * GH;
     load_G_resident(G_s, Gb, P, GH, RGH, a.vecS, tid);
-    const int t0 = a.t0, t1 = a.t1 > 0 ? a.t1 : a.T;
+    const int t0 = a.t0, t1 = a.nlive ? min(a.t1 > 0 ? a.t1 : a.T, a.nlive[b]) : (a.t1 > 0 ? a.t1 : a.T);
     for (int k = tid; k < H; k += NT) {
         h_s[k] = t0 == 0 ? a.h0[(size_t)b * H + k] : (a.Hsrc ? a.Hsrc : a.Hs)[((size_t)b * T + t0 - 1) * H + k];
         va_s[k] = a.v_a[k];
@@ -260,10 +260,17 @@
 
     const float* Gb = a.G + (size_t)b * P * GH;
     load_G_resident(G_s, Gb, P, GH, RGH, a.vecS, tid);
-    const int bt0 = a.t0, bt1 = a.t1 > 0 ? a.t1 : T;
+    const int bt0 = a.t0, wt1 = a.t1 > 0 ? a.t1 : T;
+    const int bt1 = a.nlive ? min(wt1, a.nlive[b]) : wt1;
+    for (int t = max(bt1, bt0); t < wt1; ++t) {
+        const size_t bt = (size_t)b * T + t;
+        for (int j = tid; j < GH; j += NT) { a.dgi[bt * GH + j] = 0.f; if (!LSTM) a.dgh[bt * GH + j] = 0.f; }
+        for (int k = tid; k < H; k += NT) a.duah[bt * H + k] = 0.f;
+        for (int p = tid; p < P; p += NT) a.de[bt * P + p] = 0.f;
+    }
     for (int k = tid; k < H; k += NT) {
         dh_s[k] = 0.f; va_s[k] = a.v_a[k];
-        dc_s[k] = (LSTM && bt1 < T) ? a.dc0[(size_t)b * H + k] : 0.f;
+        dc_s[k] = (LSTM && wt1 < T) ? a.dc0[(size_t)b * H + k] : 0.f;
     }
     const float* Waf_b = a.Waf + (size_t)b * P * H;
     const int CH = a.vecW ? 4 : 1;
@@ -431,6 +438,7 @@
 __global__ void attn_param_grads_kernel(AttnGradArgs a) {
     const int b = blockIdx.x, pc = blockIdx.y;
     const int P = a.P, H = a.H, T = a.T;
+    const int TL = a.nlive ? min(T, a.nlive[b]) : T;
     const int p0 = pc * a.pchunk, p1 = min(P, p0 + a.pchunk);
     const size_t blk = (size_t)b * gridDim.y + pc;
     for (int k = threadIdx.x; k < H; k += blockDim.x) {
@@ -440,7 +448,7 @@
             const float w = a.Waf[((size_t)b * P + p) * H + k];
             float s = 0.f;
 #pragma unroll 4
-            for (int t = 0; t < T; ++t) {
+            for (int t = 0; t < TL; ++t) {
                 const float de = a.de[((size_t)b * T + t) * P + p];
                 const float tv = caphn_tanh(w + a.uah[((size_t)b * T + t) * H + k]);
                 s += de * (1.0f - tv * tv);
@@ -453,7 +461,7 @@
     if (threadIdx.x == 0) {
         float s = 0.f;
         for (int p = p0; p < p1; ++p)
-            for (int t = 0; t < T; ++t) s += a.de[((size_t)b * T + t) * P + p];
+            for (int t = 0; t < TL; ++t) s += a.de[((size_t)b * T + t) * P + p];
         a.part[blk * (H + 1) + H] = s;
     }
 }
@@ -480,8 +488,9 @@
 }
 
 __global__ void ctx_kernel(int P, int F, int T, const float* __restrict__ alphas, const float* __restrict__ f, float* __restrict__ ctx,
-                           int ldc) {
+                           int ldc, const int* __restrict__ nlive) {
     const int b = blockIdx.x, t = blockIdx.y;
+    if (nlive && t >= nlive[b]) return;
     const float* al = alphas + ((size_t)b * T + t) * P;
     for (int k = threadIdx.x; k < F; k += blockDim.x) {
         float s = 0.f;
@@ -498,20 +507,23 @@
     }
 }
 __global__ void df_kernel(int P, int F, int T, const float* __restrict__ alphas, const float* __restrict__ dctx,
-                          const float* __restrict__ dmean, const float* __restrict__ dmean2, float* __restrict__ df) {
+                          const float* __restrict__ dmean, const float* __restrict__ dmean2, float* __restrict__ df,
+                          const int* __restrict__ nlive) {
     const int b = blockIdx.x, p = blockIdx.y;
     const float invP = 1.0f / (float)P;
+    const int Trow = T;
+    if (nlive) T = min(T, nlive[b]);
     for (int k = threadIdx.x; k < F; k += blockDim.x) {
         float s = (dmean2 ? dmean[(size_t)b * F + k] + dmean2[(size_t)b * F + k] : dmean[(size_t)b * F + k]) * invP;
         int t = 0;
         for (; t + 8 <= T; t += 8) {
             float a[8], v[8];
 #pragma unroll
-            for (int u = 0; u < 8; ++u) { a[u] = alphas[((size_t)b * T + t + u) * P + p]; v[u] = dctx[((size_t)b * T + t + u) * F + k]; }
+            for (int u = 0; u < 8; ++u) { a[u] = alphas[((size_t)b * Trow + t + u) * P + p]; v[u] = dctx[((size_t)b * Trow + t + u) * F + k]; }
 #pragma unroll
             for (int u = 0; u < 8; ++u) s += a[u] * v[u];
         }
-        for (; t < T; ++t) s += alphas[((size_t)b * T + t) * P + p] * dctx[((size_t)b * T + t) * F + k];
+        for (; t < T; ++t) s += alphas[((size_t)b * Trow + t) * P + p] * dctx[((size_t)b * Trow + t) * F + k];
         df[((size_t)b * P + p) * F + k] = s;
     }
 }
@@ -630,13 +642,13 @@
     hipLaunchKernelGGL(dmean_kernel, dim3(B), dim3(256), sizeof(float) * 2 * H, s, H, F, dh0, Wh, dc0, Wc, out);
     return caphn_launch_status();
 }
-int caphn_launch_ctx(int B, int T, int P, int F, const float* alphas, const float* f, float* ctx, int ldc, hipStream_t s) {
-    hipLaunchKernelGGL(ctx_kernel, dim3(B, T), dim3(F >= 192 ? 256 : 64), 0, s, P, F, T, alphas, f, ctx, ldc);
+int caphn_launch_ctx(int B, int T, int P, int F, const float* alphas, const float* f, float* ctx, int ldc, hipStream_t s, const int* nlive) {
+    hipLaunchKernelGGL(ctx_kernel, dim3(B, T), dim3(F >= 192 ? 256 : 64), 0, s, P, F, T, alphas, f, ctx, ldc, nlive);
     return caphn_launch_status();
 }
 int caphn_launch_df(int B, int T, int P, int F, const float* alphas, const float* dctx, const float* dmean, float* df, hipStream_t s,
-                    const float* dmean2) {
-    hipLaunchKernelGGL(df_kernel, dim3(B, P), dim3(F >= 192 ? 256 : 64), 0, s, P, F, T, alphas, dctx, dmean, dmean2, df);
+                    const float* dmean2, const int* nlive) {
+    hipLaunchKernelGGL(df_kernel, dim3(B, P), dim3(F >= 192 ? 256 : 64), 0, s, P, F, T, alphas, dctx, dmean, dmean2, df, nlive);
     return caphn_launch_status();
 }
 int caphn_launch_init_state(int B, int P, int F, int H, const float* f, const float* Wh, const float* bh, const float* Wc,
diff --git a/hypernet-image-captioning_amd/csrc/recurrent_pair.hip b/hypernet-image-captioning_amd/csrc/recurrent_pair.hip
--- a/hypernet-image-captioning_amd/csrc/recurrent_pair.hip
+++ b/hypernet-image-captioning_amd/csrc/recurrent_pair.hip
@@ -271,7 +271,7 @@
             G_s[(size_t)pq * nk + kk] = Gb[(size_t)p * GH + q * H + k0 + kk];
         }
     }
-    const int t0 = a.t0, t1 = a.t1 > 0 ? a.t1 : a.T, T = a.T;
+    const int T = a.T, t0 = a.t0, t1 = a.nlive ? min(a.t1 > 0 ? a.t1 : T, a.nlive[b]) : (a.t1 > 0 ? a.t1 : T);
     for (int k = tid; k < H; k += NT)
         h_s[k] = t0 == 0 ? a.h0[(size_t)b * H + k] : (a.Hsrc ? a.Hsrc : a.Hs)[((size_t)b * T + t0 - 1) * H + k];
     for (int kk = tid; kk < nk; kk += NT) {
@@ -524,10 +524,21 @@
             G_s[(size_t)pq * nk + kk] = Gb[(size_t)p * GH + q * H + k0 + kk];
         }
     }
-    const int bt0 = a.t0, bt1 = a.t1 > 0 ? a.t1 : T;
+    const int bt0 = a.t0, wt1 = a.t1 > 0 ? a.t1 : T;
+    const int bt1 = a.nlive ? min(wt1, a.nlive[b]) : wt1;
+    for (int t = max(bt1, bt0); t < wt1; ++t) {
+        const size_t bt = (size_t)b * T + t;
+        for (int j = tid; j < NG * nk; j += NT) {
+            const int q = j / nk, kk = j - q * nk;
+            a.dgi[bt * GH + q * H + k0 + kk] = 0.f;
+            if (!LSTM) a.dgh[bt * GH + q * H + k0 + kk] = 0.f;
+        }
+        for (int kk = tid; kk < nk; kk += NT) a.duah[bt * H + k0 + kk] = 0.f;
+        if (hh == 0) for (int p = tid; p < P; p += NT) a.de[bt * P + p] = 0.f;
+    }
     for (int kk = tid; kk < nk; kk += NT) {
         dh_s[kk] = 0.f; va_s[kk] = a.v_a[k0 + kk];
-        dc_s[kk] = (LSTM && bt1 < T) ? a.dc0[(size_t)b * H + k0 + kk] : 0.f;
+        dc_s[kk] = (LSTM && wt1 < T) ? a.dc0[(size_t)b * H + k0 + kk] : 0.f;
     }
     const float* Waf_b = a.Waf + (size_t)b * P * H;
     const int CH = (H % 4) == 0 ? 4 : 1;
@@ -667,7 +678,7 @@
             else { pf[5] = a.hn[bt * H + k]; pf[6] = a.Hprev[bt * H + k]; }
         }
     };
-    if (pfk) prefetch(bt1 - 1);
+    if (pfk && bt1 > bt0) prefetch(bt1 - 1);
 
     for (int t = bt1 - 1; t >= bt0; --t) {
         const size_t bt = (size_t)b * T + t;
diff --git a/include/caphn.h b/include/caphn.h
--- a/include/caphn.h
+++ b/include/caphn.h
@@ -140,6 +140,7 @@
 int caphn_decoder_pair_prep(const caphn_decoder_dims* d, const caphn_decoder_params* p, void* ws, caphn_stream_t stream);
 int caphn_decoder_pair_pack_desc(const caphn_decoder_dims* d, void* ws, caphn_pair_pack* out);
 const int* caphn_decoder_rowcount_ptr(const caphn_decoder_dims* d, void* ws);
+const int* caphn_decoder_stepmap_ptr(const caphn_decoder_dims* d, void* ws, const int** nlive_out);
 int caphn_decoder_prepare_rows(const caphn_decoder_dims* d, const int64_t* targets, int64_t ignore_index,
                                void* ws, caphn_stream_t stream);
 unsigned long long* caphn_decoder_profile_ptr(const caphn_decoder_dims* d, void* ws);
```

Result: faster. 84240 images/s (median of 6 runs) (+4.9%).
